# fabioiuri/DRecPy

Hardware: AMD Instinct MI355X
Metric: training samples/sec (user-item pairs) (higher is better)
Workload: dtype f32; 1 GPU; CDAE hidden_factors=128 sampled-output sparse-Adagrad on synth-10m-shaped synthetic (10000000 users x 1000000 items, 199573906 positives), corruption 0.2, neg_ratio 5; batch_per_gpu=65536, global_batch=65536, touch_list=prepared ahead on a side stream, batches=fresh device-sampled batch every step (sampler running ahead on the side stream)

## Files before the change

### drecpy_amd/_lib.py

```python
import ctypes as C
import os

_HERE = os.path.dirname(os.path.abspath(__file__))
LIB_PATH = os.path.join(_HERE, 'libdrx.so')

LOSS_BCE, LOSS_MSE = 0, 1
TARGETS_REFERENCE, TARGETS_PER_ROW = 0, 1
OPT_ADAM, OPT_ADAGRAD, OPT_ROWWISE_ADAGRAD = 0, 1, 2
DENSE_AUX_CLEAN = 0x100
KEY_NONE = 0xFFFFFFFF
SHARD_SELF_BYPASS = 1
BATCH_SHARE_USERS = 1


class DrxError(RuntimeError):
    pass


DRX_REC_SIGMOID_BIAS, DRX_REC_BIAS, DRX_REC_CLIP = 0, 1, 2

KNN_METRICS = {'cosine': 0, 'adjusted_cosine': 1, 'cosine_cf': 2, 'jaccard': 3, 'msd': 4, 'pearson': 5}
KNN_USER, KNN_ITEM = 0, 1
KNN_AGGREGATIONS = {'mean': 0, 'weighted_mean': 1}

# ... 69 lines not shown

class NcfDims(C.Structure):
    _fields_ = [(n, C.c_int32) for n in ('n_users', 'n_items', 'kg', 'km', 'ldg', 'ldm', 'n_layers')] + \
               [('f', C.c_int32 * 4), ('off_w', C.c_int32 * 4), ('off_b', C.c_int32 * 4), ('off_h', C.c_int32), ('off_b0', C.c_int32),
                ('n_small', C.c_int32)]


class CsrList(C.Structure):
    _fields_ = [('keys', C.c_void_p), ('T', C.c_int32), ('n_rows', C.c_int32), ('row_ptr', C.c_void_p), ('order', C.c_void_p)]


class DmfDims(C.Structure):
    _fields_ = [('n_layers', C.c_int32 * 2), ('f', (C.c_int32 * 4) * 2), ('ld0', C.c_int32 * 2),
                ('off_k', (C.c_int32 * 4) * 2), ('off_b', (C.c_int32 * 4) * 2), ('n_small', C.c_int32),
                ('l2_norm_vectors', C.c_int32), ('off_scale', C.c_int32)]


class DmfArgs(C.Structure):
    _fields_ = [(n, C.c_void_p) for n in ('K0u', 'K0i', 'sw', 'u_indptr', 'u_indices', 'u_values', 'i_indptr', 'i_indices',
                                          'i_values', 'uid', 'iid', 'y')] + [('target_mode', C.c_int32), ('y_mean', C.c_float)] + \
               [(n, C.c_void_p) for n in ('off_u', 'off_i')] + [('B', C.c_int32)] + \
               [(n, C.c_void_p) for n in ('dz0u', 'dz0i', 'tkeys_u', 'tsrc_u', 'tcoef_u', 'tkeys_i', 'tsrc_i', 'tcoef_i',
                                          'gsw_part', 'loss_part', 'pred_out', 'rep_u_out', 'rep_i_out', 'work', 'inv_u', 'inv_i',
                                          'gptr_u', 'gptr_i', 'grows_u', 'grows_i')] + [('n_du', C.c_int32), ('n_di', C.c_int32)] + \
               [(n, C.c_void_p) for n in ('map_u', 'map_i', 'rho_u', 'rho_i')] + [('stamp', C.c_uint32)] + \
               [(n, C.c_void_p) for n in ('nd_dev', 'y_mean_dev', 'work_order')] + [('n_work', C.c_int32), ('seg_len', C.c_int32)] + \
               [(n, C.c_void_p) for n in ('zseg', 'zpart', 'n_work_dev')]


class DmfK0Update(C.Structure):
    _fields_ = [(n, C.c_void_p) for n in ('K0u', 'm_u', 'v_u', 'K0i', 'm_i', 'v_i')] + [('n_items', C.c_int32), ('n_users', C.c_int32)] + \
               [(n, C.c_float) for n in ('alpha_u', 'alpha_i', 'l2_coef', 'beta1', 'beta2', 'eps')] + [('row_order', C.c_void_p), ('n_long', C.c_int32), ('opt_kind', C.c_int32)]


class Optim(C.Structure):
    _fields_ = [('kind', C.c_int32), ('lr', C.c_float), ('reg_rate', C.c_float), ('beta1', C.c_float),
                ('beta2', C.c_float), ('eps', C.c_float), ('alpha', C.c_float * 5),
                ('s1', C.c_void_p * 5), ('s2', C.c_void_p * 5)]


_lib = None

SIGNATURES = {
    'drx_version': (C.c_int, []),
    'drx_strerror': (C.c_char_p, [C.c_int]),
    'drx_hash_u32': (C.c_uint32, [C.c_uint64, C.c_uint32, C.c_uint32]),
    'drx_event_create': (C.c_void_p, []),
    'drx_event_destroy': (None, [C.c_void_p]),
    'drx_event_record': (C.c_int, [C.c_void_p, C.c_void_p]),
    'drx_stream_wait_event': (C.c_int, [C.c_void_p, C.c_void_p]),
    'drx_event_synchronize': (C.c_int, [C.c_void_p]),
    'drx_stream_create_cu_slice': (C.c_void_p, [C.c_int32]),
    'drx_stream_destroy': (None, [C.c_void_p]),
    'drx_cdae_forward': (C.c_int, [C.POINTER(CdaeParams), C.POINTER(History), C.POINTER(Batch), C.c_void_p,
                                   C.c_void_p, C.c_void_p]),
    'drx_cdae_scratch_bytes': (C.c_size_t, [C.POINTER(CdaeParams), C.c_int32, C.c_int32, C.c_int32]),
    'drx_cdae_step_dense': (C.c_int, [C.POINTER(CdaeParams), C.POINTER(Optim), C.POINTER(History), C.POINTER(Batch),
                                      C.c_int32, C.c_int32, C.c_void_p, C.c_size_t, C.c_void_p, C.c_void_p]),
    'drx_cdae_step_sparse': (C.c_int, [C.POINTER(CdaeParams), C.POINTER(Optim), C.POINTER(History), C.POINTER(Batch),
                                       C.c_int32, C.c_void_p, C.c_size_t, C.c_void_p, C.c_void_p]),
    'drx_cdae_step_sparse_timed': (C.c_int, [C.POINTER(CdaeParams), C.POINTER(Optim), C.POINTER(History),
                                             C.POINTER(Batch), C.c_int32, C.c_void_p, C.c_size_t, C.c_void_p,
                                             C.POINTER(C.c_void_p), C.c_void_p]),
    'drx_cdae_prep_bytes': (C.c_size_t, [C.POINTER(CdaeParams), C.c_int32, C.c_int32]),
    'drx_cdae_sparse_prepare': (C.c_int, [C.POINTER(CdaeParams), C.POINTER(History), C.POINTER(Batch), C.c_void_p,
                                          C.c_size_t, C.c_void_p]),
    'drx_cdae_step_sparse_prepared': (C.c_int, [C.POINTER(CdaeParams), C.POINTER(Optim), C.POINTER(History),
                                                C.POINTER(Batch), C.c_int32, C.c_void_p, C.c_size_t, C.c_void_p,
                                                C.c_size_t, C.c_void_p, C.POINTER(C.c_void_p), C.c_void_p]),
    'drx_cdae_prep_bytes_hot': (C.c_size_t, [C.POINTER(CdaeParams), C.c_int32, C.c_int32, C.c_int32]),
    'drx_cdae_scratch_bytes_hot': (C.c_size_t, [C.POINTER(CdaeParams), C.c_int32, C.c_int32, C.c_int32]),
    'drx_cdae_sparse_prepare_hot': (C.c_int, [C.POINTER(CdaeParams), C.POINTER(History), C.POINTER(Batch), C.POINTER(HotHead),
                                              C.c_void_p, C.c_size_t, C.c_void_p]),
    'drx_debug_prep_counts': (C.c_int, [C.POINTER(CdaeParams), C.POINTER(History), C.POINTER(Batch), C.POINTER(HotHead), C.c_void_p,
                                        C.c_int32, C.c_int32, C.c_int32, C.c_void_p, C.c_size_t, C.c_void_p, C.c_void_p, C.c_void_p,
                                        C.c_void_p, C.c_void_p, C.POINTER(C.c_int32), C.c_void_p]),
    'drx_debug_prep_result': (C.c_int, [C.POINTER(CdaeParams), C.c_int32, C.c_int32, C.c_int32, C.c_void_p, C.c_size_t, C.c_void_p,
                                        C.c_void_p, C.c_void_p, C.c_void_p, C.c_void_p, C.c_void_p]),
    'drx_debug_cdae_reduce': (C.c_int, [C.POINTER(CdaeParams), C.POINTER(Optim), C.POINTER(History), C.POINTER(Batch), C.POINTER(HotHead),
                                        C.c_void_p, C.c_size_t, C.c_void_p, C.c_void_p, C.c_void_p, C.c_int32, C.c_void_p, C.c_size_t,
                                        C.c_void_p]),
    'drx_debug_span_plan': (C.c_int, [C.POINTER(CdaeParams), C.c_int32, C.c_int32, C.c_int32, C.c_void_p, C.c_size_t, C.c_void_p,
                                      C.c_void_p, C.c_void_p, C.c_void_p]),
    'drx_cdae_step_sparse_hot': (C.c_int, [C.POINTER(CdaeParams), C.POINTER(Optim), C.POINTER(History), C.POINTER(Batch),
                                           C.POINTER(HotHead), C.c_int32, C.c_void_p, C.c_size_t, C.c_void_p, C.c_size_t,
                                           C.c_void_p, C.POINTER(C.c_void_p), C.c_void_p]),
    'drx_cdae_hot_rows_for': (C.c_int32, [C.POINTER(CdaeParams), C.c_int32, C.c_int32, C.c_int32, C.c_int32]),
    'drx_cdae_prep_forget': (None, [C.c_void_p]),
    'drx_point_sample_scratch_bytes': (C.c_size_t, [C.c_int32]),
    'drx_list_sample_device': (C.c_int, [C.POINTER(ListGroups), C.c_int32, C.c_int32, C.c_int32, C.c_int32, C.c_uint64, C.c_void_p, C.c_void_p,
                                         C.c_void_p, C.c_void_p]),
    'drx_point_sample': (C.c_int, [C.POINTER(History), C.c_int32, C.c_int32, C.c_int32, C.c_int32, C.c_uint64,
                                   C.c_void_p, C.c_void_p, C.c_void_p, C.c_void_p, C.c_void_p, C.c_size_t, C.c_void_p, C.c_uint32,
                                   C.c_void_p]),
    'drx_point_sample_recorded': (C.c_int, [C.POINTER(History), C.POINTER(History), C.c_int32, C.c_int32, C.c_int32, C.c_int32, C.c_uint64,
                                   C.c_void_p, C.c_void_p, C.c_void_p, C.c_void_p, C.c_void_p, C.c_size_t, C.c_void_p, C.c_uint32,
                                   C.c_void_p]),
    'drx_point_sample_by_user_scratch_bytes': (C.c_size_t, [C.c_int32, C.c_int32]),
    'drx_point_sample_by_user': (C.c_int, [C.POINTER(History), C.POINTER(History), C.c_int32, C.c_int32, C.c_int32, C.c_int32, C.c_uint64,
                                           C.c_void_p, C.c_void_p, C.c_void_p, C.c_void_p, C.c_void_p, C.c_size_t, C.c_void_p, C.c_uint32,
                                           C.c_void_p]),
    'drx_point_sample_valued': (C.c_int, [C.POINTER(History), C.POINTER(History), C.c_void_p, C.c_float, C.c_float, C.c_int32, C.c_int32,
                                          C.c_int32, C.c_int32, C.c_uint64, C.c_void_p, C.c_void_p, C.c_void_p, C.c_void_p]),
    'drx_dmf_distinct_scratch_bytes': (C.c_size_t, [C.c_int32, C.c_int32, C.c_int32]),
    'drx_dmf_batch_distinct_device': (C.c_int, [C.c_void_p, C.c_void_p, C.c_void_p, C.c_int32, C.c_int32, C.c_int32] + [C.c_void_p] * 10 +
                                      [C.c_void_p, C.c_size_t, C.c_void_p]),
    'drx_shard_prep_bytes': (C.c_size_t, [C.POINTER(CdaeParams), C.POINTER(Shard), C.c_int32, C.c_int32]),
    'drx_shard_work_bytes': (C.c_size_t, [C.POINTER(Shard)]),
    'drx_shard_prep_layout': (C.c_int, [C.POINTER(CdaeParams), C.POINTER(Shard), C.c_int32, C.c_int32, C.POINTER(C.c_size_t)]),
    'drx_shard_prepare': (C.c_int, [C.POINTER(CdaeParams), C.POINTER(Shard), C.POINTER(History), C.POINTER(Batch), C.c_void_p,
                                    C.c_size_t, C.c_void_p, C.c_size_t, C.c_void_p]),
    'drx_shard_owner_table_bytes': (C.c_size_t, [C.POINTER(Shard), C.c_int32]),
    'drx_shard_chunks': (C.c_int32, [C.POINTER(Shard)]),
    'drx_shard_unit_shift': (C.c_int32, [C.POINTER(Shard)]),
    'drx_shard_owner_index': (C.c_int, [C.POINTER(Shard), C.c_void_p, C.c_int32, C.POINTER(C.c_int32), C.c_int32, C.c_int32, C.c_void_p,
                                        C.c_size_t, C.c_void_p]),
    'drx_shard_gather_rows': (C.c_int, [C.POINTER(CdaeParams), C.POINTER(Shard), C.c_void_p, C.c_int32, C.POINTER(C.c_int32),
                                        C.c_int32, C.c_void_p, C.c_void_p]),
    'drx_shard_step_scratch_bytes': (C.c_size_t, [C.POINTER(CdaeParams), C.c_int32, C.c_int32]),
    'drx_shard_step_local': (C.c_int, [C.POINTER(CdaeParams), C.POINTER(Optim), C.POINTER(Shard), C.POINTER(History), C.POINTER(Batch),
                                       C.c_void_p, C.c_size_t, C.c_void_p, C.c_void_p, C.c_int32, C.c_int32, C.c_void_p, C.c_size_t,
                                       C.POINTER(C.c_void_p), C.c_void_p]),
    'drx_shard_apply': (C.c_int, [C.POINTER(CdaeParams), C.POINTER(Optim), C.POINTER(Shard), C.c_int32, C.c_void_p, C.c_void_p,
                                  C.c_int32, C.POINTER(C.c_int32), C.c_int32, C.c_int32, C.c_void_p, C.POINTER(C.c_void_p), C.POINTER(C.c_int64),
                                  C.c_void_p, C.c_void_p]),
    'drx_shard_exchange_sizes': (C.c_int, [C.POINTER(CdaeParams), C.POINTER(Shard), C.c_void_p, C.c_void_p, C.POINTER(C.c_int64)]),
    'drx_shard_phase_layout': (C.c_int, [C.POINTER(CdaeParams), C.POINTER(Shard), C.c_void_p, C.c_void_p, C.c_int32, C.POINTER(C.c_int64)]),
    'drx_shard_phase_keys': (C.c_int, [C.POINTER(Shard), C.c_void_p, C.POINTER(ShardExchange), C.c_void_p]),
    'drx_shard_phase_rows': (C.c_int, [C.POINTER(CdaeParams), C.POINTER(Shard), C.c_void_p, C.POINTER(ShardExchange), C.c_int32, C.c_void_p]),
    'drx_shard_phase_local': (C.c_int, [C.POINTER(CdaeParams), C.POINTER(Optim), C.POINTER(Shard), C.POINTER(History), C.POINTER(Batch),
                                        C.c_void_p, C.POINTER(ShardExchange), C.c_void_p, C.c_size_t, C.c_int32, C.c_int32, C.c_void_p,
                                        C.c_size_t, C.POINTER(C.c_void_p), C.c_void_p]),
    'drx_shard_phase_tail': (C.c_int, [C.POINTER(CdaeParams), C.POINTER(Optim), C.POINTER(Shard), C.c_void_p, C.POINTER(ShardExchange),
                                       C.POINTER(ShardExchange), C.c_int32, C.c_void_p, C.c_void_p]),
    'drx_copy_f4': (C.c_int, [C.c_void_p, C.c_void_p, C.c_size_t, C.c_void_p]),
    'drx_copy_f4_variant': (C.c_int, [C.c_void_p, C.c_void_p, C.c_size_t, C.c_int32, C.c_void_p]),
    'drx_comm_unique_id': (C.c_int, [C.c_void_p]),
    'drx_comm_create': (C.c_int, [C.c_void_p, C.c_int32, C.c_int32, C.c_uint32, C.POINTER(C.c_void_p)]),
    'drx_comm_destroy': (C.c_int, [C.c_void_p]),
    'drx_comm_stream': (C.c_void_p, [C.c_void_p]),
    'drx_comm_alltoallv': (C.c_int64, [C.c_void_p, C.c_void_p, C.POINTER(C.c_int64), C.POINTER(C.c_int64), C.c_void_p, C.POINTER(C.c_int64),
                                       C.POINTER(C.c_int64), C.c_void_p]),
    'drx_comm_wait': (C.c_int, [C.c_void_p, C.c_int64, C.c_void_p]),
    'drx_comm_last_error': (C.c_char_p, []),
    'drx_adam_dense': (C.c_int, [C.c_void_p, C.c_void_p, C.c_void_p, C.c_void_p, C.c_int64, C.c_float, C.c_float, C.c_float,
                                 C.c_float, C.c_float, C.c_void_p]),
    'drx_scatter_scratch_bytes': (C.c_size_t, [C.c_int32, C.c_int32, C.c_int32]),
    'drx_scatter_rows': (C.c_int, [C.c_void_p, C.c_int32, C.c_void_p, C.c_void_p, C.c_void_p, C.c_void_p, C.c_int32,
                                   C.c_int32, C.c_void_p, C.c_void_p, C.c_void_p, C.c_size_t, C.c_void_p]),
    'drx_batch_offsets': (C.c_int, [C.c_void_p, C.c_void_p, C.c_int32, C.c_void_p, C.c_void_p, C.c_size_t, C.c_void_p]),
    'drx_sumsq': (C.c_int, [C.c_void_p, C.c_int64, C.c_void_p, C.c_int32, C.c_void_p]),
    'drx_rows_dot': (C.c_int, [C.c_void_p, C.c_int32, C.c_void_p, C.c_int32, C.c_int32, C.c_void_p, C.c_void_p,
                               C.c_void_p]),
    'drx_adam_segments': (C.c_int, [C.c_void_p, C.c_void_p, C.c_void_p, C.c_void_p, C.POINTER(AdamSegments), C.c_float,
                                    C.c_float, C.c_float, C.c_void_p]),
    'drx_caser_grid': (C.c_int, [C.POINTER(CaserDims), C.c_int32]),
    'drx_caser_fwd_bwd': (C.c_int, [C.POINTER(CaserDims), C.POINTER(CaserArgs), C.c_void_p, C.c_void_p]),
    'drx_caser_step_small': (C.c_int, [C.POINTER(CaserDims), C.POINTER(CaserArgs), C.c_void_p, C.c_void_p, C.c_void_p, C.c_void_p,
                                       C.POINTER(AdamSegments), C.c_float, C.c_float, C.c_float, C.c_void_p]),
    'drx_caser_hidden': (C.c_int, [C.POINTER(CaserDims), C.POINTER(CaserArgs), C.c_void_p]),
    'drx_rows_csr_adam_multi': (C.c_int, [C.POINTER(CsrAdamTable), C.c_int32, C.c_float, C.c_float, C.c_float, C.c_void_p]),
    'drx_dmf_grid': (C.c_int, [C.c_int32]),
    'drx_dmf_work_bytes': (C.c_size_t, [C.c_int32]),
    'drx_dmf_fwd_bwd': (C.c_int, [C.POINTER(DmfDims), C.POINTER(DmfArgs), C.c_void_p, C.c_void_p]),
    'drx_dmf_step_small': (C.c_int, [C.POINTER(DmfDims), C.POINTER(DmfArgs), C.c_void_p, C.c_void_p, C.c_void_p, C.c_void_p,
                                     C.POINTER(AdamSegments), C.c_float, C.c_float, C.c_float, C.c_void_p]),
# ... 217 lines not shown
```

### drecpy_amd/csrc/drx_cdae.hip

```cpp
#include "drx_common.hpp"
#include "drx_rows.hpp"
#include "drx_segreduce.hpp"
#include <cstring>
#include "drx_scan.hpp"
#include "drx_prep.hpp"
#include "drx_segstream.hpp"
#include "drx_cdae_host.hpp"
#include <type_traits>
#include <mutex>
#include <unordered_map>

#ifdef DRX_STAMPS
static unsigned long long *h_stamps = nullptr;
extern "C" int drx_debug_set_stamps(unsigned long long *buf, unsigned int) { h_stamps = buf; return 0; }
#endif

namespace drx {

struct SparseBufs {
  float *dz1;
  float *g2;
  float *dz2;
  float *lossb;
  float *phead, *ptail;
  float *phs, *pts;
  float *pblock, *pbs;
  float *bpart;
  const uint8_t *solo_v, *solo_o;
  unsigned long long *stamps;
  const int32_t *order;
  const int32_t *usamp, *worder, *n_items;
  const WorkItem *witem;
  int T, n_chunks, n_bpart;
};

template <int G, int J, int KIND = -1>
__device__ __forceinline__ void sparse_apply(const DrxCdaeParams &P, const DrxOptim &opt, int B, uint32_t key, int lane,
                                             const float4 (&g)[J], float gs) {
  const uint32_t N = (uint32_t)P.n_items;
  float *const tW = P.W, *const tO = P.W2T, *const tV = P.V;
  float *const a0 = opt.s1[0], *const a1 = opt.s1[1], *const a2 = opt.s1[2];
  float *const c0 = opt.s2[0], *const c1 = opt.s2[1], *const c2 = opt.s2[2];
  const int var = key < N ? 0 : (key < 2 * N ? 1 : 2);
  const size_t row = key - (uint32_t)var * N;
  float *const tab = var == 0 ? tW : (var == 1 ? tO : tV);
  float *const s1 = var == 0 ? a0 : (var == 1 ? a1 : a2);
  float *const s2 = var == 0 ? c0 : (var == 1 ? c1 : c2);
  OptScalars o = opt_for(opt, 0, B);
  o.inv_k = 1.0f / (float)P.k;
  float4 w[J];
  load_row<G, J>(tab, row, P.ld, lane, w);
  row_update<G, J, KIND>(o, tab, s1, s2, row, P.ld, lane, w, g);
  if (var == 1 && lane == 0) {
    const int kind = KIND >= 0 ? KIND : o.kind;
    float pb = P.b2[row], m = opt.s1[4][row], v = kind == DRX_OPT_ADAM ? opt.s2[4][row] : 0.f;
    o.rb = 0.f;
    opt_update1<KIND>(o, gs, pb, m, v);
    P.b2[row] = pb; opt.s1[4][row] = m;
    if (kind == DRX_OPT_ADAM) opt.s2[4][row] = v;
  }
}

template <int G, int J>
__device__ __forceinline__ float sampled_hidden(const DrxCdaeParams &P, const DrxBatch &bt, float scale, int b, int lane,
                                                const float4 (&acc)[J], float4 (&h)[J], float4 (&w2)[J]) {
  hidden_act<G, J>(P, bt.uid[b], scale, lane, acc, h);
  load_row<G, J>(P.W2T, (size_t)bt.iid[b], P.ld, lane, w2);
  float d = 0.f;
#pragma unroll
  for (int j = 0; j < J; ++j) d += f4_dot(w2[j], h[j]);
  return group_sum<G>(d);
}

template <int G, int J, int KIND = -1>
__device__ __forceinline__ void sampled_rest(const DrxCdaeParams &P, const DrxOptim &opt, const DrxHistory &H, const DrxBatch &bt,
                                             float scale, uint32_t qthr, int loss_kind, const SparseBufs &S, int b, int lane,
                                             float d, const float4 (&h)[J], const float4 (&w2)[J],
                                             float4 (*dz1_out)[J] = nullptr) {
  const int u = bt.uid[b], i = bt.iid[b];
  const float y = bt.y[b];
  const float p = sigmoidf_(d + P.b2[i]);
  const float invB = 1.0f / (float)bt.B;
  float lval, dp;
  if (loss_kind == DRX_LOSS_BCE) { lval = bce_elem(y, p); dp = bce_grad(y, p) * invB; }
  else { lval = (p - y) * (p - y); dp = 2.0f * (p - y) * invB; }
  const float dz2 = dp * p * (1.0f - p);
  float4 dz1[J], g2[J];
#pragma unroll
  for (int j = 0; j < J; ++j) {
    dz1[j].x = dz2 * w2[j].x * h[j].x * (1.0f - h[j].x); dz1[j].y = dz2 * w2[j].y * h[j].y * (1.0f - h[j].y);
    dz1[j].z = dz2 * w2[j].z * h[j].z * (1.0f - h[j].z); dz1[j].w = dz2 * w2[j].w * h[j].w * (1.0f - h[j].w);
    g2[j].x = dz2 * h[j].x; g2[j].y = dz2 * h[j].y; g2[j].z = dz2 * h[j].z; g2[j].w = dz2 * h[j].w;
  }
  store_row<G, J>(S.dz1, (size_t)b, P.ld, lane, dz1);
  if (lane == 0) S.lossb[b] = lval;
  const uint8_t *const pv = S.solo_v, *const po = S.solo_o;
  const bool solo_v = pv && pv[b], solo_o = po && po[b];
  if (solo_o) {
    sparse_apply<G, J, KIND>(P, opt, bt.B, (uint32_t)P.n_items + (uint32_t)i, lane, g2, dz2);
  } else {
    store_row<G, J>(S.g2, (size_t)b, P.ld, lane, g2);
    if (lane == 0) S.dz2[b] = dz2;
  }
  if (solo_v) sparse_apply<G, J, KIND>(P, opt, bt.B, 2u * (uint32_t)P.n_items + (uint32_t)u, lane, dz1, 0.f);
  if (dz1_out) {
#pragma unroll
    for (int j = 0; j < J; ++j) (*dz1_out)[j] = dz1[j];
  }
}

template <int G, int J, int KIND = -1>
__device__ __forceinline__ void sampled_finish(const DrxCdaeParams &P, const DrxOptim &opt, const DrxHistory &H, const DrxBatch &bt,
                                               float scale, uint32_t qthr, int loss_kind, const SparseBufs &S, int b, int lane,
                                               const float4 (&acc)[J]) {
  float4 h[J], w2[J];
#ifdef DRX_STAMPS
  if (acc[0].x == acc[0].x) DRX_STAMP(S.stamps, b, 5, lane);
#endif
  const float d = sampled_hidden<G, J>(P, bt, scale, b, lane, acc, h, w2);
#ifdef DRX_STAMPS
  if (d == d) DRX_STAMP(S.stamps, b, 6, lane);
#endif
  sampled_rest<G, J, KIND>(P, opt, H, bt, scale, qthr, loss_kind, S, b, lane, d, h, w2);
  DRX_STAMP(S.stamps, b, 7, lane);
}

template <int G, int J>
__global__ __launch_bounds__(kBlock) void k_kshard_fwd(DrxCdaeParams P, DrxHistory H, DrxBatch bt, float scale, uint32_t qthr,
                                                       float *__restrict__ h_out, float *__restrict__ dot_out,
                                                       const int32_t *__restrict__ order) {
  const int lane = threadIdx.x % G;
  const int slot = blockIdx.x * (kBlock / G) + threadIdx.x / G;
  if (slot >= bt.B) return;
  const int b = order ? order[slot] : slot;
  float4 acc[J], h[J], w2[J];
  DenseAux none{};
  gather_bag<G, J, 0>(P, H, bt, qthr, b, lane, acc, none, nullptr, nullptr, 0);
  const float d = sampled_hidden<G, J>(P, bt, scale, b, lane, acc, h, w2);
  store_row<G, J>(h_out, (size_t)b, P.ld, lane, h);
  if (lane == 0) dot_out[b] = d;
}

// ... 156 lines not shown
      for (int wv = 0; wv < n_waves; ++wv) {
        float4 x[J];
        load_row<G, J>(lds, (size_t)(wv * RT + t), P.ld, lane, x);
#pragma unroll
        for (int j = 0; j < J; ++j) f4_add(acc[j], x[j]);
      }
      float4 brow[J];
      load_row<G, J>(P.b, 0, P.ld, lane, brow);
      hidden_act_rows<G, J>(P, scale, lane, acc, vrow, brow, h);
      load_row<G, J>(P.W2T, (size_t)bt.iid[b], P.ld, lane, w2);
      float d = 0.f;
#pragma unroll
      for (int j = 0; j < J; ++j) d += f4_dot(w2[j], h[j]);
      d = group_sum<G>(d);
      sampled_rest<G, J, KIND>(P, opt, H, bt, scale, qthr, loss_kind, S, b, lane, d, h, w2, &dz1);
#pragma unroll
      for (int j = 0; j < J; ++j) f4_add(dsum[j], dz1[j]);
    }
  }
  __syncthreads();
  if (r < n) store_row<G, J>(lds, (size_t)r, P.ld, lane, dsum);
  __syncthreads();
  if (r == 0) {
    float4 t[J];
#pragma unroll
    for (int j = 0; j < J; ++j) t[j] = f4_zero();
    for (int rr = 0; rr < min(n, R); ++rr) {
      float4 x[J];
      load_row<G, J>(lds, (size_t)rr, P.ld, lane, x);
#pragma unroll
      for (int j = 0; j < J; ++j) f4_add(t[j], x[j]);
    }
    store_row<G, J>(S.dz1, (size_t)bt.B + w, P.ld, lane, t);
  }
}

template <int G, int J>
__global__ __launch_bounds__(kBlock) void k_sampled_fwd_bwd_wg(DrxCdaeParams P, DrxOptim opt, DrxHistory H, DrxBatch bt, float scale,
                                                               uint32_t qthr, int loss_kind, SparseBufs S) {
  extern __shared__ __align__(16) float lds[];
  constexpr int R = kBlock / G;
  const int lane = threadIdx.x % G, r = threadIdx.x / G;
  const int b = blockIdx.x;
  float4 acc[J];
  DenseAux none{};
  gather_bag<G, J, 0>(P, H, bt, qthr, b, lane, acc, none, nullptr, nullptr, 0, r, R);
  store_row<G, J>(lds, (size_t)r, P.ld, lane, acc);
  __syncthreads();
  if (r != 0) return;
#pragma unroll
  for (int j = 0; j < J; ++j) acc[j] = f4_zero();
#pragma unroll 8
  for (int rr = 0; rr < R; ++rr) {
    float4 v[J];
    load_row<G, J>(lds, (size_t)rr, P.ld, lane, v);
#pragma unroll
    for (int j = 0; j < J; ++j) f4_add(acc[j], v[j]);
  }
  sampled_finish<G, J>(P, opt, H, bt, scale, qthr, loss_kind, S, b, lane, acc);
}

template <int KIND>
struct DirectPolicyT {
  DrxCdaeParams P;
  DrxOptim opt;
  int B;
  float scale;
  const float *dz1;
  long long g2_off;
  const float *dz2;
  template <int G, int J>
  __device__ __forceinline__ void load(uint32_t key, uint32_t bv, int lane, float4 (&row)[J], float &sc, float &coef) const {
    const uint32_t N = (uint32_t)P.n_items;
    const bool is_out = key >= N && key < 2 * N;
    const uint32_t b = bv & 0x7FFFFFFFu;
    load_row<G, J>(dz1 + (is_out ? g2_off : 0ll), (size_t)b, P.ld, lane, row);
    if (is_out) sc = dz2[b];
    coef = key < N ? ((bv >> 31) ? -scale : scale) : 1.0f;
  }
  template <int G, int J>
  __device__ __forceinline__ void finish(uint32_t key, int, int lane, const float4 (&g)[J], float gs) const {
    sparse_apply<G, J, KIND>(P, opt, B, key, lane, g, gs);
  }
  static constexpr bool kStreamParks = false;
  __device__ __forceinline__ StreamArrays stream_arrays() const {
    const uint32_t N = (uint32_t)P.n_items;
    return StreamArrays{{0u, N, 2u * N}, {dz1, dz1 + g2_off, dz1}, {P.W, P.W2T, P.V}, {opt.s1[0], opt.s1[1], opt.s1[2]},
                        {scale, 1.0f, 1.0f}, {nullptr, dz2, nullptr}, {nullptr, P.b2, nullptr}, {nullptr, opt.s1[4], nullptr}};
  }
  __device__ __forceinline__ float stream_decay() const { return opt.reg_rate / (float)B; }
  __device__ __forceinline__ void stream_update(float g, float &p, float &a) const {
    static_assert(KIND == DRX_OPT_ADAGRAD || KIND < 0, "one slot per element");
    OptScalars o = opt_for(opt, 0, B);
    float unused = 0.f;
    opt_update1<DRX_OPT_ADAGRAD>(o, g, p, a, unused);
  }
  __device__ __forceinline__ void stream_update_scalar(float g, float &p, float &a) const { stream_update(g, p, a); }
};
using DirectPolicy = DirectPolicyT<-1>;
using DirectPolicyAdagrad = DirectPolicyT<DRX_OPT_ADAGRAD>;

template <int G, int J, int NT>
__device__ __forceinline__ void bias_final_body(const DrxCdaeParams &P, const DrxOptim &opt, const BiasArgs &A,
                                                float *lds , float *red) {
  constexpr int R = NT / G;
  const int lane = threadIdx.x % G, r = threadIdx.x / G;
  float4 acc[J];
#pragma unroll
  for (int j = 0; j < J; ++j) acc[j] = f4_zero();
  constexpr int NB = J == 1 ? 8 : 2;
  for (int i = r; i < A.n_part; i += NB * R) {
    float4 v[NB][J];
#pragma unroll
    for (int q = 0; q < NB; ++q) {
#pragma unroll
      for (int j = 0; j < J; ++j) v[q][j] = f4_zero();
      if (i + q * R < A.n_part) load_row<G, J>(A.part, (size_t)(i + q * R), P.ld, lane, v[q]);
    }
#pragma unroll
    for (int q = 0; q < NB; ++q)
#pragma unroll
      for (int j = 0; j < J; ++j) f4_add(acc[j], v[q][j]);
  }
  store_row<G, J>(lds, (size_t)r, P.ld, lane, acc);
  __syncthreads();
  if (r == 0) {
    float4 g[J], w[J];
#pragma unroll
    for (int j = 0; j < J; ++j) g[j] = f4_zero();
#pragma unroll 8
    for (int rr = 0; rr < R; ++rr) {
      float4 v[J];
      load_row<G, J>(lds, (size_t)rr, P.ld, lane, v);
#pragma unroll
      for (int j = 0; j < J; ++j) f4_add(g[j], v[j]);
    }
    load_row<G, J>(P.b, 0, P.ld, lane, w);
    OptScalars o = opt_for(opt, 0, A.B);
    if (o.kind == DRX_OPT_ROWWISE_ADAGRAD) o.kind = DRX_OPT_ADAGRAD;
    o.rb = 0.f;
    row_update<G, J>(o, P.b, opt.s1[3], opt.s2[3], 0, P.ld, lane, w, g);
  }
  if (A.loss_out) {
    const float *lp = A.part + (size_t)A.n_part * P.ld;
    float a = 0.f;
    for (int b = threadIdx.x; b < A.n_part; b += NT) a += lp[b];
    float t = block_sum(a, red);
    if (threadIdx.x == 0) { A.loss_out[0] = t / (float)A.B; A.loss_out[1] = 0.f; }
  }
}

template <int G, int J>
struct BiasFinalExtra {
  DrxCdaeParams P;
  DrxOptim opt;
  BiasArgs A;
  __device__ __forceinline__ void operator()(float *lds) const {
    __shared__ float red[kFixBlock / 64];
    bias_final_body<G, J, kFixBlock>(P, opt, A, lds, red);
  }
};

constexpr int kHotSlice = 512;
constexpr int kHotGroup = 64;

struct HotArgs {
  const float *dz1;
  const uint32_t *mask;
  float *part;
  uint32_t *any;
  const int32_t *item;
  float scale;
  int B, H, Bw, S, first;
  float *bpart;
  const float *lossb;
};

static inline int hot_slices(int B) { return (B + kHotSlice - 1) / kHotSlice; }
static inline int hot_groups(int H) { return (H + kHotGroup - 1) / kHotGroup; }

typedef __bf16 hot_bf16x8 __attribute__((ext_vector_type(8)));
typedef float hot_f32x4 __attribute__((ext_vector_type(4)));
typedef uint32_t hot_u32x4 __attribute__((ext_vector_type(4)));

template <int LD, int NT>
struct HotPartialExtra {
  HotArgs A;
  __device__ __forceinline__ void operator()(float *) const {
    constexpr int CS = LD / 16, NW = NT / 64;
    const int lane = threadIdx.x & 63, wv = __builtin_amdgcn_readfirstlane((int)(threadIdx.x >> 6));
    const int ngr = (A.H + kHotGroup - 1) / kHotGroup;
    const int task = ((int)blockIdx.x - A.first) * NW + wv;
    if (task >= A.S * ngr * CS) return;
    const int cs = task % CS, rg = (task / CS) % ngr, s = task / (CS * ngr);
    const int c = lane & 15, kq = lane >> 4;
    const int nt = min(kHotGroup, A.H - rg * kHotGroup) / 16;
    const int b_begin = s * kHotSlice, b_end = min(A.B, b_begin + kHotSlice);
    const uint32_t *const mgrp = A.mask + (size_t)rg * kHotGroup * A.Bw;
    const float *const slice = A.dz1 + (size_t)b_begin * LD + cs * 16;
    const uint32_t mlane = (uint32_t)c * (uint32_t)A.Bw, xlane = (uint32_t)(8 * kq * LD + c);
    hot_f32x4 acc[4];
#pragma unroll
    for (int t = 0; t < 4; ++t) acc[t] = hot_f32x4{0.f, 0.f, 0.f, 0.f};
    uint32_t seen = 0u;
    float bsum = 0.f;
    for (int b0 = b_begin; b0 < b_end; b0 += 32) {
      float x[8];
      uint32_t w[4];
      {
        const float *const rows = slice + (size_t)(b0 - b_begin) * LD;
        const uint32_t *const words = mgrp + (b0 >> 5);
        const int left = A.B - b0 - 8 * kq;
        if (left >= 8) {
#pragma unroll
          for (int j = 0; j < 8; ++j) x[j] = rows[xlane + (uint32_t)(j * LD)];
        } else {
#pragma unroll
          for (int j = 0; j < 8; ++j) x[j] = j < left ? rows[xlane + (uint32_t)(j * LD)] : 0.f;
        }
#pragma unroll
        for (int t = 0; t < 4; ++t) w[t] = (words + (size_t)(16 * min(t, nt - 1)) * A.Bw)[mlane] & (t < nt ? ~0u : 0u);
      }
      hot_u32x4 bh, bm, bl;
#pragma unroll
      for (int i = 0; i < 4; ++i) {
        uint32_t hv[2], mv[2], lv[2];
#pragma unroll
        for (int e = 0; e < 2; ++e) {
          const float v = x[2 * i + e];
          bsum += v;
          hv[e] = __float_as_uint(v) & 0xFFFF0000u;
          const float r1 = v - __uint_as_float(hv[e]);
          mv[e] = __float_as_uint(r1) & 0xFFFF0000u;
          lv[e] = __float_as_uint(r1 - __uint_as_float(mv[e])) & 0xFFFF0000u;
        }
        bh[i] = (hv[0] >> 16) | hv[1];
        bm[i] = (mv[0] >> 16) | mv[1];
        bl[i] = (lv[0] >> 16) | lv[1];
      }
#pragma unroll
      for (int t = 0; t < 4; ++t) {
        seen |= (w[t] != 0u ? 1u : 0u) << t;
        const uint32_t bits = (w[t] >> (8 * kq)) & 0xFFu;
        hot_u32x4 a;
#pragma unroll
        for (int i = 0; i < 4; ++i) a[i] = ((bits >> (2 * i)) & 1u) * 0x3F80u | ((bits >> (2 * i + 1)) & 1u) * 0x3F800000u;
        const hot_bf16x8 av = __builtin_bit_cast(hot_bf16x8, a);
        acc[t] = __builtin_amdgcn_mfma_f32_16x16x32_bf16(av, __builtin_bit_cast(hot_bf16x8, bh), acc[t], 0, 0, 0);
        acc[t] = __builtin_amdgcn_mfma_f32_16x16x32_bf16(av, __builtin_bit_cast(hot_bf16x8, bm), acc[t], 0, 0, 0);
        acc[t] = __builtin_amdgcn_mfma_f32_16x16x32_bf16(av, __builtin_bit_cast(hot_bf16x8, bl), acc[t], 0, 0, 0);
      }
    }
    float *const out = A.part + ((size_t)s * A.H + rg * kHotGroup) * LD + cs * 16 + c;
#pragma unroll
    for (int t = 0; t < 4; ++t)
      if (t < nt) {
#pragma unroll
        for (int i = 0; i < 4; ++i) out[(size_t)(16 * t + 4 * kq + i) * LD] = acc[t][i];
      }
    if (cs == 0) {
      uint32_t rows[4];
#pragma unroll
      for (int t = 0; t < 4; ++t) rows[t] = (uint32_t)__ballot((seen >> t) & 1u) & 0xFFFFu;
      if (lane == 0) {
        uint32_t *const any = A.any + (size_t)s * (A.H / 32) + rg * (kHotGroup / 32);
        any[0] = rows[0] | (rows[1] << 16);
        if (nt > 2) any[1] = rows[2] | (rows[3] << 16);
      }
    }
    if (rg == 0) {
      const float g1 = __shfl(bsum, c + 16, 64), g2 = __shfl(bsum, c + 32, 64), g3 = __shfl(bsum, c + 48, 64);
      if (kq == 0) A.bpart[(size_t)s * LD + cs * 16 + c] = ((bsum + g1) + g2) + g3;
      if (cs == 0 && A.lossb) {
        float l = 0.f;
        for (int b = b_begin + lane; b < b_end; b += 64) l += A.lossb[b];
#pragma unroll
        for (int o = 32; o > 0; o >>= 1) l += __shfl_xor(l, o, 64);
        if (lane == 0) A.bpart[(size_t)A.S * LD + s] = l;
      }
    }
  }
};

template <int LD, class Policy>
struct HotFinishExtra {
  HotArgs A;
  Policy pol;
  __device__ __forceinline__ void operator()(float *lds) const {
    constexpr int NT = kFixBlock, NQ = NT / LD;
    static_assert(NQ >= 1 && NT % LD == 0, "a row per workgroup");
    const int h = (int)blockIdx.x - A.first;
    if (h >= A.H) return;
    const uint32_t bit = 1u << (h & 31);
    bool touched = false;
    for (int s = (int)threadIdx.x; s < A.S; s += NT) touched |= (A.any[(size_t)s * (A.H / 32) + (h >> 5)] & bit) != 0u;
    if (!__syncthreads_or(touched)) return;
    const int c = (int)threadIdx.x % LD, q = (int)threadIdx.x / LD;
    const int per = (A.S + NQ - 1) / NQ, s0 = q * per, s1 = min(A.S, s0 + per);
    float sum = 0.f;
#pragma unroll 8
    for (int s = s0; s < s1; ++s) sum += A.part[((size_t)s * A.H + h) * LD + c];
    lds[q * LD + c] = sum;
    __syncthreads();
    if (q == 0) {
      float t = lds[c];
#pragma unroll
      for (int k = 1; k < NQ; ++k) t += lds[k * LD + c];
      const StreamArrays SA = pol.stream_arrays();
      const size_t off = (size_t)A.item[h] * LD + c;
      float pv = SA.table[0][off], av = SA.slot[0][off];
      pol.stream_update(fmaf(pol.stream_decay(), pv, A.scale * t), pv, av);
      SA.table[0][off] = pv;
      SA.slot[0][off] = av;
    }
  }
};

template <class E1, class E2>
struct ExtraPair {
  E1 e1;
  int n1;
  E2 e2;
  __device__ __forceinline__ void operator()(float *lds) const {
    if ((int)blockIdx.x < n1) e1(lds);
    else e2(lds);
  }
};

static SparseBufs sparse_layout(Carver &cv, const DrxCdaeParams &P, int B, int n_touch_slots) {
  SparseBufs S{};
  S.T = n_touch_slots + 2 * B;
  const int chunk = seg_chunk(long_segments(S.T, P));
  S.n_chunks = (S.T + chunk - 1) / chunk;
  S.n_bpart = 1024;
  S.dz1 = cv.take<float>((size_t)2 * B * P.ld);
  S.g2 = cv.take<float>((size_t)B * P.ld);
  S.dz2 = cv.take<float>(B);
  S.lossb = cv.take<float>(B);
  S.phead = cv.take<float>((size_t)S.n_chunks * P.ld);
  S.ptail = cv.take<float>((size_t)S.n_chunks * P.ld);
  S.phs = cv.take<float>(S.n_chunks);
  S.pts = cv.take<float>(S.n_chunks);
  {
    const int cpb = kSegBlock / pick_geom(P.ld).G;
    const int n_blocks = (S.n_chunks + cpb - 1) / cpb;
    S.pblock = cv.take<float>((size_t)n_blocks * P.ld);
    S.pbs = cv.take<float>(n_blocks);
  }
  S.bpart = cv.take<float>((size_t)S.n_bpart * (P.ld + 1));
  return S;
}

static std::mutex g_hot_mu;
static std::unordered_map<const void *, int> g_hot_of;
static void hot_record(const void *prepared, int H) {
  std::lock_guard<std::mutex> lk(g_hot_mu);
  if (H > 0) g_hot_of[prepared] = H;
  else g_hot_of.erase(prepared);
}
static int hot_recorded(const void *prepared) {
  std::lock_guard<std::mutex> lk(g_hot_mu);
  const auto it = g_hot_of.find(prepared);
  return it == g_hot_of.end() ? 0 : it->second;
}

struct HotBufs { float *part; uint32_t *any; float *bpart; };
static HotBufs hot_layout(Carver &cv, const DrxCdaeParams &P, int B, int H) {
  HotBufs HB{nullptr, nullptr, nullptr};
  if (H <= 0) return HB;
  HB.part = cv.take<float>((size_t)hot_slices(B) * H * P.ld);
  HB.any = cv.take<uint32_t>((size_t)hot_slices(B) * (H / 32));
  HB.bpart = cv.take<float>((size_t)hot_slices(B) * (P.ld + 1));
  return HB;
}

template <int G, int J>
static void launch_forward(ForwardForm form, const DrxCdaeParams &P, const DrxOptim &opt, const DrxHistory &hist, const DrxBatch &bt,
                           float scale, uint32_t qthr, int32_t loss_kind, const SparseBufs &S, const float *ks_h, const float *ks_dot,
                           hipStream_t st) {
  constexpr int gpb = kBlock / G;
  const dim3 groups((bt.B + gpb - 1) / gpb);
  const bool adagrad = opt.kind == DRX_OPT_ADAGRAD;
  switch (form) {
  case ForwardForm::ColumnShard:
    hipLaunchKernelGGL((k_kshard_rest<G, J>), groups, dim3(kBlock), 0, st, P, opt, hist, bt, scale, qthr, loss_kind, S, ks_h, ks_dot);
    break;
  case ForwardForm::SharedUsers:
    if constexpr (G >= 16 && J <= 2) {
      const long long wmax = (long long)(P.n_users < bt.B ? P.n_users : bt.B) + bt.B / share_item_triples(P.ld) + 1;
      hipLaunchKernelGGL((adagrad ? k_items_fwd_bwd<G, J, DRX_OPT_ADAGRAD> : k_items_fwd_bwd<G, J>), dim3((unsigned)(wmax < bt.B ? wmax : bt.B)),
                         dim3(kItemThreads), share_item_lds_bytes(P.ld), st, P, opt, hist, bt, scale, qthr, loss_kind, S);
    }
    break;
  case ForwardForm::PerWorkgroup:
    hipLaunchKernelGGL((k_sampled_fwd_bwd_wg<G, J>), dim3(bt.B), dim3(kBlock), (size_t)gpb * P.ld * 4, st, P, opt, hist, bt, scale, qthr,
                       loss_kind, S);
    break;
  case ForwardForm::PerGroup:
    hipLaunchKernelGGL((adagrad ? k_sampled_fwd_bwd<G, J, DRX_OPT_ADAGRAD> : k_sampled_fwd_bwd<G, J>), groups, dim3(kBlock), 0, st, P, opt, hist,
                       bt, scale, qthr, loss_kind, S);
    break;
  }
}

template <int G, int J, class Policy>
static int reduce_and_finish(ReduceForm form, const DrxCdaeParams &P, const DrxOptim &opt, const SparseBufs &S, const SegBufs &SB,
                             const PlanBufs &PB, const SpanPlan &plan, const BiasArgs &BA, const HotArgs &HA, void *const *events,
                             hipStream_t st) {
  const Policy pol{P, opt, BA.B, HA.scale, S.dz1, (long long)(S.g2 - S.dz1), S.dz2};
  const BiasFinalExtra<G, J> bias{P, opt, BA};
  int rc = DRX_EINVAL;
  if (HA.H == 0) rc = launch_reduce<G, J>(form, SB, PB, plan, pol, BA, st);
  else if constexpr (kHotBuilt<G, J, Policy>) {
    constexpr int NT = kStreamThreads<G>;
    HotArgs part = HA;
    part.first = 0;
    const int n_hot = (HA.S * hot_groups(HA.H) * (G / 4) + NT / 64 - 1) / (NT / 64);
    rc = launch_reduce_streamed<G, J>(SB, PB, plan, pol, n_hot, HotPartialExtra<4 * G, NT>{part}, st);
  }
  if (rc) return rc;
  DRX_HIP(phase_event(events, 3, st));
  rc = DRX_EINVAL;
  if (HA.H == 0) rc = launch_spans<G, J>(SB, PB, plan, pol, 1, bias, st);
  else if constexpr (kHotBuilt<G, J, Policy>) {
    HotArgs fin = HA;
    fin.first = kSpanBlocks + 1;
    using Finish = ExtraPair<BiasFinalExtra<G, J>, HotFinishExtra<4 * G, Policy>>;
    rc = launch_spans<G, J>(SB, PB, plan, pol, 1 + HA.H, Finish{bias, fin.first, {fin, pol}}, st);
  }
  if (rc) return rc;
  DRX_HIP(phase_event(events, 4, st));
  DRX_HIP(phase_event(events, 5, st));
  return DRX_OK;
}

}

using namespace drx;

extern "C" {

size_t drx_cdae_scratch_bytes(const DrxCdaeParams *p, int32_t B, int32_t n_touch_slots, int32_t dense_mode) {
  if (!p || B < 1 || n_touch_slots < 0) return 0;
  Carver c(nullptr, 0);
  if (dense_mode) {
    c.off = dense_layout_bytes(*p, B);
  } else {
    (void)sparse_layout(c, *p, B, n_touch_slots);
    (void)prep_layout(c, *p, B, n_touch_slots);
  }
  return align_up(c.off, 256) + 256;
}

struct GivenGradients { const float *dz1, *g2, *dz2; int32_t form; };

static int step_sparse_impl(const DrxCdaeParams *p, const DrxOptim *opt, const DrxHistory *hist, const DrxBatch *bt,
                            int32_t loss_kind, const void *prepared, size_t prepared_bytes, void *scratch, size_t scratch_bytes,
                            float *loss_out, void *const *events, void *stream, const float *ks_h = nullptr,
                            const float *ks_dot = nullptr, const DrxHotHead *hot = nullptr, const GivenGradients *given = nullptr) {
  int rc = check_params(p);
  if (rc) return rc;
  rc = check_batch(hist, bt);
  if (rc || !opt || !scratch || !bt->iid || (!bt->y && !given) || !bt->keep_off) return DRX_EINVAL;
  if (opt->kind != DRX_OPT_ADAM && opt->kind != DRX_OPT_ADAGRAD && opt->kind != DRX_OPT_ROWWISE_ADAGRAD) return DRX_EINVAL;
  for (int i = 0; i < 5; ++i)
    if (!opt->s1[i] || (opt->kind == DRX_OPT_ADAM && !opt->s2[i])) return DRX_EINVAL;
  if ((uint64_t)2 * p->n_items + p->n_users + 1 >= 0xFFFFFFFFull) return DRX_EINVAL;
  hipStream_t st = (hipStream_t)stream;
  const int H = hot ? hot->H : 0;
  if (prepared && hot_recorded(prepared) != H) return DRX_EINVAL;
  Carver cv(scratch, scratch_bytes);
  SparseBufs S = sparse_layout(cv, *p, bt->B, bt->n_touch_slots);
  const HotBufs HB = hot_layout(cv, *p, bt->B, H);
  PrepBufs R{};
  if (prepared) {
    Carver cp(const_cast<void *>(prepared), prepared_bytes);
    R = prep_layout(cp, *p, bt->B, bt->n_touch_slots, H);
    if (!cp.ok()) return DRX_ESCRATCH;
  } else {
    R = prep_layout(cv, *p, bt->B, bt->n_touch_slots, H);
  }
  if (!cv.ok()) return DRX_ESCRATCH;
  const float scale = 1.0f / (1.0f - bt->q);
  const uint32_t qthr = q_threshold(bt->q);
  const int rows_per_block = (bt->B + S.n_bpart - 1) / S.n_bpart;
  const int n_bpart = (bt->B + rows_per_block - 1) / rows_per_block;
  S.solo_v = prepared ? R.solo_v : nullptr;
  S.solo_o = prepared ? R.solo_o : nullptr;
  S.order = prepared ? R.order : nullptr;
  SegBufs SB{R.keys_s, R.vals_s, S.phead, S.ptail, S.phs, S.pts, nullptr, nullptr, nullptr, nullptr, S.T, S.n_chunks, p->ld, nullptr};
#ifdef DRX_STAMPS
  S.stamps = SB.stamps = h_stamps;
#endif
  PlanBufs PB{S.pblock, S.pbs};
  if (prepared && ks_h && share_users(p, hist, bt, R)) return DRX_EINVAL;
  const bool share = prepared && !ks_h && share_users(p, hist, bt, R);
  S.usamp = share ? R.usamp : nullptr;
  S.witem = share ? R.witem : nullptr;
  S.worder = share ? R.worder : nullptr;
  S.n_items = share ? R.n_du : nullptr;
  ReduceForm form = reduce_form(opt->kind, bt->B, S.T, *p);
  const ForwardForm fwd = forward_form(ks_h != nullptr, share, bt->B, bt->n_touch_slots);
  if (H > 0 && !hot_head_fits(form, p->ld, share, ks_h != nullptr)) return DRX_EINVAL;
  if (given) {
    if (share || (given->form == 1 && (H > 0 || form == ReduceForm::PlannedLong))) return DRX_EINVAL;
    if (given->form == 1) form = ReduceForm::PlannedShort;
  }
  const HotArgs HA{S.dz1, R.hmask, HB.part, HB.any, hot ? hot->item : nullptr, scale, bt->B, H, R.Bw, hot_slices(bt->B), 0, HB.bpart,
                   loss_out ? S.lossb : nullptr};
// ... 169 lines not shown

int drx_debug_prep_counts(const DrxCdaeParams *p, const DrxHistory *hist, const DrxBatch *bt, const DrxHotHead *hot, uint8_t *present,
                          int32_t ipr, int32_t cshift, int32_t world, void *prepared, size_t prepared_bytes, uint32_t *hist_out,
                          uint32_t *buckets_out, uint32_t *keys_out, uint32_t *vals_out, uint32_t *mask_out, int32_t *info_out,
                          void *stream) {
  int rc = check_params(p);
  if (rc) return rc;
  rc = check_batch(hist, bt);
  if (rc || !prepared || !bt->iid || !bt->keep_off || !hist_out || !buckets_out || !keys_out || !vals_out || !info_out) return DRX_EINVAL;
  if ((uint64_t)2 * p->n_items + p->n_users + 1 >= 0xFFFFFFFFull) return DRX_EINVAL;
  if (hot && !hot_ok(p, hot)) return DRX_EINVAL;
  if (present && (ipr < 1 || cshift < 0 || cshift > 30 || world < 1)) return DRX_EINVAL;
  const int H = hot ? hot->H : 0;
  if (H > 0 && !mask_out) return DRX_EINVAL;
  Carver cp(prepared, prepared_bytes);
  const PrepBufs R = prep_layout(cp, *p, bt->B, bt->n_touch_slots, H);
  if (!cp.ok()) return DRX_ESCRATCH;
  if (H > 0 && !hot_list_fits(R.T, *p, present != nullptr)) return DRX_EINVAL;
  hipStream_t st = (hipStream_t)stream;
  hot_record(prepared, 0);
  launch_touches(p, hist, bt, R, st, TouchPresence{present, WireGeo{present ? ipr : 1, present ? cshift : 0, present ? world : 1}},
                 H > 0 ? hot->slot : nullptr, H > 0 ? hot->item : nullptr);
  const SortRider rider{bt->keep_off, bt->B, R.order_work, R.partials, R.partial_rows};
  const uint32_t *h = nullptr;
  rc = sort_first_counts(R.sort_temp, R.sort_bytes, R.keys, (size_t)R.T, R.bits, true, st, rider, &h);
  if (rc) return rc;
  const int dbits = sort_first_digit_bits(R.bits);
  DRX_HIP(hipMemcpyAsync(hist_out, h, sizeof(uint32_t) << dbits, hipMemcpyDeviceToDevice, st));
  DRX_HIP(hipMemcpyAsync(buckets_out, R.order_work, 256 * sizeof(uint32_t), hipMemcpyDeviceToDevice, st));
  DRX_HIP(hipMemcpyAsync(keys_out, R.keys, (size_t)R.T * sizeof(uint32_t), hipMemcpyDeviceToDevice, st));
  DRX_HIP(hipMemcpyAsync(vals_out, R.vals, (size_t)R.T * sizeof(uint32_t), hipMemcpyDeviceToDevice, st));
  if (H > 0) DRX_HIP(hipMemcpyAsync(mask_out, R.hmask, (size_t)H * R.Bw * sizeof(uint32_t), hipMemcpyDeviceToDevice, st));
  info_out[0] = dbits;
  info_out[1] = R.partials ? R.partial_rows : 0;
  info_out[2] = R.T;
  info_out[3] = DRX_PREP_ROUNDS ? touch_grid(bt->B) : (bt->B + 15) / 16;
  DRX_LAUNCH_CHECK();
  return DRX_OK;
}

int drx_debug_prep_result(const DrxCdaeParams *p, int32_t B, int32_t n_touch_slots, int32_t H, const void *prepared, size_t prepared_bytes,
                          uint32_t *keys_s_out, uint32_t *vals_s_out, uint8_t *solo_v_out, uint8_t *solo_o_out, int32_t *order_out,
                          void *stream) {
  int rc = check_params(p);
  if (rc) return rc;
  if (B < 1 || n_touch_slots < 0 || hot_rows(p, H) < 0 || !prepared || !keys_s_out || !vals_s_out || !solo_v_out || !solo_o_out || !order_out)
    return DRX_EINVAL;
  Carver cp(const_cast<void *>(prepared), prepared_bytes);
  const PrepBufs R = prep_layout(cp, *p, B, n_touch_slots, H);
  if (!cp.ok()) return DRX_ESCRATCH;
  hipStream_t st = (hipStream_t)stream;
  DRX_HIP(hipMemcpyAsync(keys_s_out, R.keys_s, (size_t)R.T * sizeof(uint32_t), hipMemcpyDeviceToDevice, st));
  DRX_HIP(hipMemcpyAsync(vals_s_out, R.vals_s, (size_t)R.T * sizeof(uint32_t), hipMemcpyDeviceToDevice, st));
  DRX_HIP(hipMemcpyAsync(solo_v_out, R.solo_v, (size_t)B, hipMemcpyDeviceToDevice, st));
  DRX_HIP(hipMemcpyAsync(solo_o_out, R.solo_o, (size_t)B, hipMemcpyDeviceToDevice, st));
  DRX_HIP(hipMemcpyAsync(order_out, R.order, (size_t)B * sizeof(int32_t), hipMemcpyDeviceToDevice, st));
  return DRX_OK;
}

int drx_debug_cdae_reduce(const DrxCdaeParams *p, const DrxOptim *opt, const DrxHistory *hist, const DrxBatch *bt, const DrxHotHead *hot,
                          const void *prepared, size_t prepared_bytes, const float *dz1_in, const float *g2_in, const float *dz2_in,
                          int32_t form, void *scratch, size_t scratch_bytes, void *stream) {
  if (!dz1_in || !g2_in || !dz2_in || (form != 0 && form != 1) || (hot && !hot_ok(p, hot))) return DRX_EINVAL;
  const GivenGradients given{dz1_in, g2_in, dz2_in, form};
  return step_sparse_impl(p, opt, hist, bt, DRX_LOSS_BCE, prepared, prepared_bytes, scratch, scratch_bytes, nullptr, nullptr, stream,
                          nullptr, nullptr, hot && hot->H > 0 ? hot : nullptr, &given);
}

int drx_debug_span_plan(const DrxCdaeParams *p, int32_t B, int32_t n_touch_slots, int32_t H, const void *prepared, size_t prepared_bytes,
                        uint8_t *ext_out, uint32_t *desc_out, uint32_t *cnt_out, void *stream) {
  int rc = check_params(p);
  if (rc) return rc;
  if (B < 1 || n_touch_slots < 0 || hot_rows(p, H) < 0 || !prepared || !ext_out || !desc_out || !cnt_out) return DRX_EINVAL;
  Carver cp(const_cast<void *>(prepared), prepared_bytes);
  const PrepBufs R = prep_layout(cp, *p, B, n_touch_slots, H);
  if (!cp.ok()) return DRX_ESCRATCH;
  hipStream_t st = (hipStream_t)stream;
  DRX_HIP(hipMemcpyAsync(ext_out, R.plan.ext, (size_t)R.n_chunks, hipMemcpyDeviceToDevice, st));
  DRX_HIP(hipMemcpyAsync(desc_out, R.plan.desc, (size_t)R.n_chunks * sizeof(uint2), hipMemcpyDeviceToDevice, st));
  DRX_HIP(hipMemcpyAsync(cnt_out, R.plan.cnt, 2 * sizeof(uint32_t), hipMemcpyDeviceToDevice, st));
  return DRX_OK;
}

int drx_cdae_step_sparse_hot(const DrxCdaeParams *p, const DrxOptim *opt, const DrxHistory *hist, const DrxBatch *bt,
                             const DrxHotHead *hot, int32_t loss_kind, const void *prepared, size_t prepared_bytes, void *scratch,
                             size_t scratch_bytes, float *loss_out, void *const *events, void *stream) {
  if (!hot_ok(p, hot)) return DRX_EINVAL;
  return step_sparse_impl(p, opt, hist, bt, loss_kind, prepared, prepared_bytes, scratch, scratch_bytes, loss_out, events, stream,
                          nullptr, nullptr, hot);
}

int32_t drx_cdae_hot_rows_for(const DrxCdaeParams *p, int32_t opt_kind, int32_t B, int32_t n_touch_slots, int32_t H) {
  if (B < 1 || n_touch_slots < 0 || hot_rows(p, H) <= 0) return 0;
  return hot_head_fits(reduce_form(opt_kind, B, n_touch_slots + 2 * B, *p), p->ld, false, false) ? H : 0;
}

void drx_cdae_prep_forget(const void *prepared) {
  if (prepared) hot_record(prepared, 0);
}

}
```

### drecpy_amd/csrc/drx_common.hpp

```cpp
#pragma once
#include <cstring>
#include <hip/hip_runtime.h>
#include <stdint.h>
#include "drx.h"

#define DRX_HIP(expr)                                  \
  do {                                                 \
    hipError_t e_ = (expr);                            \
    if (e_ != hipSuccess) return (int)e_;              \
  } while (0)

#define DRX_LAUNCH_CHECK()                             \
  do {                                                 \
    hipError_t e_ = hipGetLastError();                 \
    if (e_ != hipSuccess) return (int)e_;              \
  } while (0)

namespace drx {

constexpr int kWave = 64;
constexpr int kBlock = 256;

__host__ __device__ inline uint32_t hash_u32(uint64_t seed, uint32_t a, uint32_t b) {
  uint64_t x = seed + (uint64_t)a * 0x9E3779B97F4A7C15ull + (uint64_t)b * 0xD1B54A32D192ED03ull;
// ... 1 lines not shown
  x ^= x >> 27; x *= 0x94D049BB133111EBull;
  x ^= x >> 31;
  return (uint32_t)(x >> 32);
}

__host__ __device__ inline uint32_t q_threshold(float q) {
  double t = (double)q * 4294967296.0;
  if (t <= 0.0) return 0u;
  if (t >= 4294967295.0) return 0xFFFFFFFFu;
  return (uint32_t)t;
}

template <int G>
__device__ __forceinline__ float group_sum(float v) {
#pragma unroll
  for (int m = G / 2; m >= 1; m >>= 1) v += __shfl_xor(v, m, kWave);
  return v;
}

__device__ __forceinline__ float4 f4_zero() { return make_float4(0.f, 0.f, 0.f, 0.f); }
__device__ __forceinline__ void f4_fma(float4 &a, float s, const float4 &x) {
  a.x = fmaf(s, x.x, a.x); a.y = fmaf(s, x.y, a.y); a.z = fmaf(s, x.z, a.z); a.w = fmaf(s, x.w, a.w);
}
__device__ __forceinline__ void f4_add(float4 &a, const float4 &x) {
  a.x += x.x; a.y += x.y; a.z += x.z; a.w += x.w;
}
__device__ __forceinline__ float f4_dot(const float4 &a, const float4 &b) {
  return fmaf(a.x, b.x, fmaf(a.y, b.y, fmaf(a.z, b.z, a.w * b.w)));
}

__device__ __forceinline__ float sigmoidf_(float x) { return 1.0f / (1.0f + expf(-x)); }

__device__ __forceinline__ float bce_elem(float t, float p) {
  const float eps = 1e-7f;
  float pc = fminf(fmaxf(p, eps), 1.0f - eps);
  return -(t * logf(pc + eps) + (1.0f - t) * logf(1.0f - pc + eps));
}
__device__ __forceinline__ float bce_grad(float t, float p) {
  const float eps = 1e-7f;
  float pc = fminf(fmaxf(p, eps), 1.0f - eps);
  float g = -(t / (pc + eps) - (1.0f - t) / (1.0f - pc + eps));
  return (p >= eps && p <= 1.0f - eps) ? g : 0.0f;
}

struct Geom { int G, J; };
inline Geom pick_geom(int ld) {
  if (ld <= 16) return {4, 1};
  if (ld <= 32) return {8, 1};
  if (ld <= 64) return {16, 1};
  if (ld <= 128) return {32, 1};
  if (ld <= 256) return {64, 1};
  if (ld <= 512) return {64, 2};
  return {64, 4};
}

template <int G_, int J_> struct GeomT { static constexpr int G = G_, J = J_; };

template <class F>
inline int dispatch_geom(int ld, F &&f) {
  const Geom g = pick_geom(ld);
  if (g.G == 4) return f(GeomT<4, 1>{});
  if (g.G == 8) return f(GeomT<8, 1>{});
  if (g.G == 16) return f(GeomT<16, 1>{});
  if (g.G == 32) return f(GeomT<32, 1>{});
  if (g.J == 1) return f(GeomT<64, 1>{});
  if (g.J == 2) return f(GeomT<64, 2>{});
  return f(GeomT<64, 4>{});
}

__device__ __forceinline__ void wave_lds_sync() {
  __builtin_amdgcn_fence(__ATOMIC_RELEASE, "workgroup");
  __builtin_amdgcn_wave_barrier();
  __builtin_amdgcn_fence(__ATOMIC_ACQUIRE, "workgroup");
}

#ifdef DRX_STAMPS
#define DRX_STAMP(buf, unit, i, lane)                                                             \
  do {                                                                                            \
    if ((lane) == 0 && (buf) && (unsigned)(unit) < 110000u) (buf)[(size_t)(unit) * 16 + (i)] = wall_clock64(); \
  } while (0)
#else
#define DRX_STAMP(buf, unit, i, lane) do { } while (0)
#endif

inline size_t align_up(size_t x, size_t a) { return (x + a - 1) / a * a; }

struct Carver {
  char *base; size_t off; size_t cap;
  Carver(void *p, size_t c) : base((char *)p), off(0), cap(c) {}
  template <typename T> T *take(size_t n) {
    off = align_up(off, 256);
    T *r = (T *)(base ? base + off : nullptr);
    off += n * sizeof(T);
    return r;
  }
  bool ok() const { return off <= cap; }
};

size_t sort_pairs_temp_bytes(size_t n, int end_bit);
int sort_pairs(void *temp, size_t temp_bytes, const uint32_t *kin, uint32_t *kout, const uint32_t *vin,
               uint32_t *vout, size_t n, int end_bit, hipStream_t stream);
__device__ __forceinline__ int degree_bucket(const int32_t *keep_off, int b) {
  const int d = (keep_off[b + 1] - keep_off[b]) >> 2;
  return 255 - (d > 255 ? 255 : d);
}

__device__ __forceinline__ unsigned long long same_bucket_lanes(bool valid, int d) {
  unsigned long long m = __ballot(valid);
#pragma unroll
  for (int bit = 0; bit < 8; ++bit) {
    const bool one = (d >> bit) & 1;
    const unsigned long long bl = __ballot(one);
    m &= one ? bl : ~bl;
  }
  return m;
}

template <int NT>
__device__ __forceinline__ void degree_counts_body(const int32_t *__restrict__ keep_off, int B, unsigned int *__restrict__ work, int block_id,
                                                   unsigned int *cnt ) {
  for (int i = threadIdx.x; i < 256; i += NT) cnt[i] = 0;
  __syncthreads();
  const int b = block_id * NT + (int)threadIdx.x, lane = threadIdx.x & 63;
  const bool valid = b < B;
  const int d = valid ? degree_bucket(keep_off, b) : 0;
  const unsigned long long m = same_bucket_lanes(valid, d);
  if (valid && lane == __ffsll((long long)m) - 1) atomicAdd(&cnt[d], (unsigned int)__popcll(m));
  __syncthreads();
  for (int i = threadIdx.x; i < 256; i += NT)
    if (cnt[i]) atomicAdd(&work[i], cnt[i]);
}

struct SortRider {
  const int32_t *keep_off;
  int B;
  unsigned int *counts;
  const uint32_t *partials = nullptr;
  int partial_rows = 0;
};
constexpr int kPartialWords = 512;
int sort_first_digit_bits(int end_bit);

int sort_pairs_ex(void *temp, size_t temp_bytes, const uint32_t *kin, uint32_t *kout, const uint32_t *vin, uint32_t *vout, size_t n, int end_bit,
                  bool drop_none, hipStream_t stream, bool pre_zeroed = false, SortRider rider = SortRider{nullptr, 0, nullptr});
void sort_pairs_zero_region(void *temp, size_t n, int end_bit, uint32_t **words, size_t *n_words);
int sort_first_counts(void *temp, size_t temp_bytes, const uint32_t *kin, size_t n, int end_bit, bool drop_none, hipStream_t stream,
                      SortRider rider, const uint32_t **hist);

inline int bits_for(uint64_t max_key_exclusive) {
  int b = 1;
  while (b < 32 && (1ull << b) < max_key_exclusive) ++b;
  return b;
}

}
```

### drecpy_amd/csrc/drx_prep.hpp

```cpp
#pragma once
#include <algorithm>
#include "drx_common.hpp"
#include "drx_rows.hpp"
#include "drx_segreduce.hpp"
#include "drx_scan.hpp"

namespace drx {

struct WireGeo {
  int ipr, cshift, world;
  __host__ __device__ __forceinline__ uint32_t wire(int item, int is_out) const {
    const int o = item / ipr;
    const uint32_t l = 2u * (uint32_t)(item - o * ipr) + (uint32_t)(is_out ? 1 : 0);
    return (((l >> cshift) * (uint32_t)world + (uint32_t)o) << cshift) | (l & ((1u << cshift) - 1u));
  }
  __host__ __device__ __forceinline__ uint32_t local(uint32_t w) const {
    return (((w >> cshift) / (uint32_t)world) << cshift) | (w & ((1u << cshift) - 1u));
  }
  __host__ __device__ __forceinline__ uint32_t unit(uint32_t w) const { return w >> cshift; }
};

struct TouchPresence {
  uint8_t *present;
  WireGeo G;
// ... 388 lines not shown
constexpr int kLongBlocks = 256, kShortBlocks = 1024;

struct __attribute__((aligned(32))) WorkItem { int32_t p0, n, user, deg; long long hist_start, pad_; };

struct PrepBufs {
  uint32_t *keys_s, *vals_s, *keys, *vals;
  void *sort_temp;
  size_t sort_bytes;
  uint8_t *solo_v, *solo_o;
  SpanPlan plan;
  int32_t *order;
  int32_t *usamp;
  int32_t *pitem;
  WorkItem *witem;
  int32_t *worder;
  int32_t *n_du;
  unsigned int *order_work;
  int n_chunks;
  size_t result_bytes;
  int T, bits;
  uint32_t *hmask;
  int H, Bw;
  uint32_t *partials;
  int partial_rows;
};

static inline bool long_segments(int T, const DrxCdaeParams &P) { return (int64_t)T > 8 * ((int64_t)2 * P.n_items + P.n_users); }

#ifndef DRX_STREAM_DEPTH
#define DRX_STREAM_DEPTH 4
#endif
constexpr int kStreamDepth = DRX_STREAM_DEPTH;
constexpr int kStreamIndexBits = 28;
constexpr int kHotMaxG = 32;

enum class ReduceForm { Streamed, PlannedLong, PlannedShort };

template <class Policy> struct PolicyKind;
template <template <int> class PolicyT, int KIND> struct PolicyKind<PolicyT<KIND>> { static constexpr int value = KIND; };
template <int G, int J, class Policy>
constexpr bool kStreamBuilt = kStreamDepth > 0 && J == 1 && G >= 16 && PolicyKind<Policy>::value == DRX_OPT_ADAGRAD;
template <int G, int J, class Policy>
constexpr bool kHotBuilt = kStreamBuilt<G, J, Policy> && G <= kHotMaxG;

static inline ReduceForm reduce_form(int opt_kind, int B, int T, const DrxCdaeParams &K) {
  if (long_segments(T, K)) return ReduceForm::PlannedLong;
  const Geom gm = pick_geom(K.ld);
  const bool streamed = kStreamDepth > 0 && gm.J == 1 && gm.G >= 16 && K.ld == 4 * gm.G && opt_kind == DRX_OPT_ADAGRAD &&
                        B < (1 << kStreamIndexBits) && K.n_items < (1 << kStreamIndexBits) && K.n_users < (1 << kStreamIndexBits);
  return streamed ? ReduceForm::Streamed : ReduceForm::PlannedShort;
}

static inline bool hot_list_fits(int T, const DrxCdaeParams &K, bool presence) { return !presence && !long_segments(T, K); }
static inline bool hot_head_fits(ReduceForm form, int ld, bool share, bool kshard) {
  return form == ReduceForm::Streamed && pick_geom(ld).G <= kHotMaxG && !share && !kshard;
}

static inline bool forward_per_workgroup(int B, int n_touch_slots) {
  const long long mean_hist = n_touch_slots / (long long)B;
  return mean_hist > 64 || (B <= 8192 && mean_hist > 16);
}
enum class ForwardForm { ColumnShard, SharedUsers, PerWorkgroup, PerGroup };
static inline ForwardForm forward_form(bool kshard, bool share, int B, int n_touch_slots) {
  if (kshard) return ForwardForm::ColumnShard;
  if (share) return ForwardForm::SharedUsers;
  return forward_per_workgroup(B, n_touch_slots) ? ForwardForm::PerWorkgroup : ForwardForm::PerGroup;
}

static inline hipError_t phase_event(void *const *events, int i, hipStream_t st) {
  return events ? hipEventRecord((hipEvent_t)events[i], st) : hipSuccess;
}

static PrepBufs prep_layout(Carver &cv, const DrxCdaeParams &P, int B, int n_touch_slots, int H = 0) {
  PrepBufs R{};
  R.T = n_touch_slots + 2 * B;
  R.bits = bits_for((uint64_t)2 * P.n_items + P.n_users + 1);
  R.keys_s = cv.take<uint32_t>(R.T);
  R.vals_s = cv.take<uint32_t>(R.T);
  R.solo_v = cv.take<uint8_t>((size_t)2 * B);
  R.solo_o = R.solo_v ? R.solo_v + B : nullptr;
  R.plan.chunk = seg_chunk(long_segments(R.T, P));
  R.n_chunks = (R.T + R.plan.chunk - 1) / R.plan.chunk;
  R.plan.desc = cv.take<uint2>(R.n_chunks);
  R.plan.cnt = cv.take<uint32_t>(128);
  R.plan.ext = cv.take<uint8_t>(R.n_chunks);
  {
    R.plan.xstride = (R.n_chunks + 1) / 2;
    const bool placed = long_segments(R.T, P);
    const bool placed_any = placed || DRX_STREAM_PLACED != 0;
    R.plan.xrank = placed_any ? cv.take<uint32_t>((size_t)R.plan.xstride) : nullptr;
    R.plan.xperm = placed_any ? cv.take<uint32_t>((size_t)R.plan.xstride) : nullptr;
    R.usamp = placed ? cv.take<int32_t>(B) : nullptr;
    R.pitem = placed ? cv.take<int32_t>(B) : nullptr;
    R.witem = placed ? cv.take<WorkItem>((size_t)B) : nullptr;
    R.worder = placed ? cv.take<int32_t>(B) : nullptr;
    R.n_du = placed ? cv.take<int32_t>(128) : nullptr;
  }
  R.order = cv.take<int32_t>(B);
  R.result_bytes = align_up(cv.off, 256);
  R.keys = cv.take<uint32_t>(R.T);
  R.vals = cv.take<uint32_t>(R.T);
  R.sort_bytes = sort_pairs_temp_bytes(R.T, R.bits);
  R.sort_temp = cv.take<char>(R.sort_bytes);
  R.order_work = cv.take<unsigned int>(512);
  R.H = H;
  R.Bw = (B + 31) / 32;
  R.hmask = H > 0 ? cv.take<uint32_t>((size_t)H * R.Bw) : nullptr;
  R.partial_rows = DRX_PREP_ROUNDS && sort_first_digit_bits(R.bits) == 8 ? touch_grid(B) : 0;
  R.partials = R.partial_rows > 0 ? cv.take<uint32_t>((size_t)R.partial_rows * kPartialWords) : nullptr;
  return R;
}

static int plan_zero_words(const PrepBufs &R) { return (int)(((const char *)R.plan.ext + R.n_chunks - (const char *)R.plan.cnt + 3) / 4); }

static int plan_spans(const DrxCdaeParams *p, const DrxBatch *bt, const PrepBufs &R0, hipStream_t st, bool cleared) {
  const PrepBufs &R = R0;
  if (!cleared) DRX_HIP(hipMemsetAsync(R.plan.cnt, 0, (size_t)plan_zero_words(R) * 4, st));
  hipLaunchKernelGGL(k_plan_spans<0>, dim3((R.n_chunks + 255) / 256), dim3(256), 0, st, R.keys_s, R.vals_s, R.T, R.n_chunks,
                     kSegBlock / pick_geom(p->ld).G, bt->B, R.plan);
  if (R.plan.xrank) hipLaunchKernelGGL(k_place_blocks, dim3(256), dim3(256), 0, st, R.plan, R.n_chunks);
  return DRX_OK;
}

static void order_by_degree(const DrxBatch *bt, const PrepBufs &R, hipStream_t st, bool cleared) {
  if (!cleared) (void)hipMemsetAsync(R.order_work, 0, 512 * sizeof(unsigned int), st);
  const int blocks = (bt->B + 1023) / 1024;
  hipLaunchKernelGGL(k_degree_counts, dim3(blocks), dim3(1024), 0, st, bt->keep_off, bt->B, R.order_work);
  hipLaunchKernelGGL(k_degree_scatter, dim3(blocks), dim3(1024), 0, st, bt->keep_off, bt->B, R.order_work, R.order);
}

constexpr int kTpFallback = 0x7fff0001;

static __global__ __launch_bounds__(256) void k_tp_begin(DrxBatch bt, int n_users, uint32_t *__restrict__ k2, uint32_t *__restrict__ v2,
                                                         int32_t *__restrict__ se, int n_se, uint8_t *solo, uint32_t *zero_a, int n_zero_a,
                                                         uint32_t *zero_b, int n_zero_b) {
  const int tid = blockIdx.x * blockDim.x + threadIdx.x, nt = gridDim.x * blockDim.x;
  for (int j = tid; j < 2 * bt.B; j += nt) {
    k2[j] = j < bt.B ? (uint32_t)bt.uid[j] : (uint32_t)n_users + (uint32_t)bt.iid[j - bt.B];
    v2[j] = (uint32_t)j;
  }
  for (int j = tid; j < n_se; j += nt) se[j] = 0;
  for (int j = tid; j < 2 * bt.B; j += nt) solo[j] = 0;
  for (int j = tid; j < n_zero_a; j += nt) zero_a[j] = 0u;
  for (int j = tid; j < n_zero_b; j += nt) zero_b[j] = 0u;
}

static __global__ __launch_bounds__(256) void k_tp_runs(const uint32_t *__restrict__ ks, int n, int32_t *__restrict__ start, int32_t *__restrict__ end) {
  for (int p = blockIdx.x * blockDim.x + threadIdx.x; p < n; p += gridDim.x * blockDim.x) {
    const uint32_t k = ks[p];
    if (p == 0 || ks[p - 1] != k) start[k] = p;
    if (p == n - 1 || ks[p + 1] != k) end[k] = p + 1;
  }
}

#ifndef DRX_ITEM_THREADS
#define DRX_ITEM_THREADS 256
#endif
constexpr int kShareTriples = 16;
static inline int share_item_triples(int) { return kShareTriples; }
constexpr int kItemThreads = DRX_ITEM_THREADS;
static inline size_t share_item_lds_bytes(int ld) { return ((size_t)(kItemThreads / 64) * kShareTriples * ld + kShareTriples) * 4; }
static inline bool share_geometry_ok(int ld) {
  const Geom g = pick_geom(ld);
  return g.G >= 16 && g.J <= 2 && share_item_lds_bytes(ld) <= 64 * 1024;
}

// ... 301 lines not shown
```

### drecpy_amd/csrc/drx_rows.hpp

```cpp
#pragma once
#include "drx_common.hpp"

#ifndef DRX_GATHER_ROWS
#define DRX_GATHER_ROWS 8
#endif
#ifndef DRX_GATHER_PACKED
#define DRX_GATHER_PACKED 1
#endif

namespace drx {

template <int G, int J>
__device__ __forceinline__ void load_row(const float *base, size_t row, int ld, int lane, float4 (&v)[J]) {
  const float4 *r = reinterpret_cast<const float4 *>(base + row * (size_t)ld);
#pragma unroll
  for (int j = 0; j < J; ++j) {
    int c = lane + j * G;
    v[j] = (4 * c < ld) ? r[c] : f4_zero();
  }
}

template <int G, int J>
__device__ __forceinline__ void store_row(float *base, size_t row, int ld, int lane, const float4 (&v)[J]) {
  float4 *r = reinterpret_cast<float4 *>(base + row * (size_t)ld);
// ... 80 lines not shown
          tvals[touch_base + jj] = (uint32_t)b;
        }
      }
    }
    constexpr int NF = J == 1 ? DRX_GATHER_ROWS : 4;
#ifdef DRX_STAMPS
    if (first_rows && idx[0] >= -1) DRX_STAMP(stamps, b, 3, lane);
#endif
    if constexpr (DRX_GATHER_PACKED != 0 && CH <= 32) {
      uint32_t left = 0;
#pragma unroll
      for (int rr = 0; rr < IPL; ++rr) left |= (uint32_t)group_ballot<G>(kf[rr] != 0) << (rr * G);
      while (left) {
        float4 r[NF][J];
#pragma unroll
        for (int q = 0; q < NF; ++q) {
          const bool on = left != 0;
          const int tt = on ? __builtin_ctz(left) : 0;
          left &= left - 1;
          int si = idx[0];
#pragma unroll
          for (int rr = 1; rr < IPL; ++rr) si = (tt / G == rr) ? idx[rr] : si;
          const int iq = __shfl(si, tt % G, G);
#pragma unroll
          for (int jx = 0; jx < J; ++jx) r[q][jx] = f4_zero();
          if (on) load_row<G, J>(P.W, (size_t)iq, P.ld, lane, r[q]);
        }
#pragma unroll
        for (int q = 0; q < NF; ++q)
#pragma unroll
          for (int jx = 0; jx < J; ++jx) f4_add(acc[jx], r[q][jx]);
#ifdef DRX_STAMPS
        if (first_rows && acc[0].x == acc[0].x) { DRX_STAMP(stamps, b, 4, lane); first_rows = false; }
#endif
      }
    } else {
      const int n_here = (int)((e - c) < (int64_t)CH ? (e - c) : (int64_t)CH);
      for (int t = 0; t < n_here; t += NF) {
        float4 r[NF][J];
#pragma unroll
        for (int q = 0; q < NF; ++q) {
          const int tt = t + q;
          int si = idx[0], sk = kf[0];
#pragma unroll
          for (int rr = 1; rr < IPL; ++rr) { si = (tt / G == rr) ? idx[rr] : si; sk = (tt / G == rr) ? kf[rr] : sk; }
          const int iq = __shfl(si, tt % G, G);
          const int kq = (tt < n_here) ? __shfl(sk, tt % G, G) : 0;
#pragma unroll
          for (int jx = 0; jx < J; ++jx) r[q][jx] = f4_zero();
          if (kq) load_row<G, J>(P.W, (size_t)iq, P.ld, lane, r[q]);
        }
#pragma unroll
        for (int q = 0; q < NF; ++q)
#pragma unroll
          for (int jx = 0; jx < J; ++jx) f4_add(acc[jx], r[q][jx]);
#ifdef DRX_STAMPS
        if (first_rows && acc[0].x == acc[0].x) { DRX_STAMP(stamps, b, 4, lane); first_rows = false; }
#endif
      }
    }
  }
}

struct OptScalars {
  int kind;
  float lr, rb;
  float b1, b2, eps, alpha;
  float inv_k = 0.f;
};

template <int KIND = -1>
__device__ __forceinline__ void opt_update1(const OptScalars &o, float g, float &p, float &s1, float &s2) {
  const int kind = KIND >= 0 ? KIND : o.kind;
  if (kind == DRX_OPT_ADAM) {
    s1 = s1 + (g - s1) * (1.0f - o.b1);
    s2 = s2 + (g * g - s2) * (1.0f - o.b2);
    p = p - (s1 * o.alpha) / (sqrtf(s2) + o.eps);
  } else {
    s1 = s1 + g * g;
    p = p - o.lr * g / (sqrtf(s1) + o.eps);
  }
}

template <int G, int J, int KIND = -1>
__device__ __forceinline__ float row_update(const OptScalars &o, float *tab, float *s1, float *s2, size_t row, int ld,
                                            int lane, const float4 (&w)[J], const float4 (&g)[J]) {
  float sq = 0.f;
  float4 *pr = reinterpret_cast<float4 *>(tab + row * (size_t)ld);
  const int kind = KIND >= 0 ? KIND : o.kind;
  if (kind == DRX_OPT_ROWWISE_ADAGRAD) {
    float4 gg[J];
    float q = 0.f;
#pragma unroll
    for (int j = 0; j < J; ++j) {
      const float4 p = w[j];
      gg[j].x = fmaf(o.rb, p.x, g[j].x); gg[j].y = fmaf(o.rb, p.y, g[j].y);
      gg[j].z = fmaf(o.rb, p.z, g[j].z); gg[j].w = fmaf(o.rb, p.w, g[j].w);
      q += f4_dot(gg[j], gg[j]);
      sq += f4_dot(p, p);
    }
    q = group_sum<G>(q) * o.inv_k;
    const float acc = s1[row * (size_t)ld] + q;
    const float step = o.lr / (sqrtf(acc) + o.eps);
#pragma unroll
    for (int j = 0; j < J; ++j) {
      const int c = lane + j * G;
      if (4 * c < ld) {
        float4 p = w[j];
        p.x -= step * gg[j].x; p.y -= step * gg[j].y; p.z -= step * gg[j].z; p.w -= step * gg[j].w;
        pr[c] = p;
      }
    }
    if (lane == 0) s1[row * (size_t)ld] = acc;
    return sq;
  }
  float4 *a1 = reinterpret_cast<float4 *>(s1 + row * (size_t)ld);
  float4 *a2 = (kind == DRX_OPT_ADAM) ? reinterpret_cast<float4 *>(s2 + row * (size_t)ld) : nullptr;
#pragma unroll
  for (int j = 0; j < J; ++j) {
    const int c = lane + j * G;
    if (4 * c < ld) {
      float4 p = w[j];
      float4 m = a1[c];
      float4 v = a2 ? a2[c] : f4_zero();
      sq += f4_dot(p, p);
      opt_update1<KIND>(o, fmaf(o.rb, p.x, g[j].x), p.x, m.x, v.x);
      opt_update1<KIND>(o, fmaf(o.rb, p.y, g[j].y), p.y, m.y, v.y);
      opt_update1<KIND>(o, fmaf(o.rb, p.z, g[j].z), p.z, m.z, v.z);
      opt_update1<KIND>(o, fmaf(o.rb, p.w, g[j].w), p.w, m.w, v.w);
      pr[c] = p;
      a1[c] = m;
      if (a2) a2[c] = v;
    }
  }
  return sq;
}

__device__ __forceinline__ OptScalars opt_for(const DrxOptim &opt, int var, int B) {
  OptScalars o;
  o.kind = opt.kind; o.lr = opt.lr; o.rb = opt.reg_rate / (float)B;
  o.b1 = opt.beta1; o.b2 = opt.beta2; o.eps = opt.eps; o.alpha = opt.alpha[var];
  return o;
}

__device__ __forceinline__ float block_sum(float v, float *red ) {
  v = group_sum<64>(v);
  __syncthreads();
  if ((threadIdx.x & 63) == 0) red[threadIdx.x >> 6] = v;
  __syncthreads();
  float t = 0.f;
  if (threadIdx.x == 0)
    for (int i = 0; i < (int)(blockDim.x >> 6); ++i) t += red[i];
  return t;
}

}
```

### drecpy_amd/csrc/drx_segreduce.hpp

```cpp
#pragma once
#include "drx_rows.hpp"

namespace drx {

#ifndef DRX_CHUNK
#define DRX_CHUNK 32
#endif
constexpr int kChunk = DRX_CHUNK;
constexpr int kChunkLong = 64;
static inline int seg_chunk(bool long_segments) { return long_segments ? kChunkLong : kChunk; }
#ifdef DRX_SEG_WAVE_PER_CHUNK
#define SEG_GPB(G) (drx::kBlock / 64)
#else
#define SEG_GPB(G) (drx::kBlock / (G))
#endif
constexpr int kShortSpan = 64;
#ifndef DRX_SEG_BLOCK
#define DRX_SEG_BLOCK 128
#endif
constexpr int kSegBlock = DRX_SEG_BLOCK;
constexpr int kPlanShort = 16;
constexpr int kFixBlock = 512;

struct SegBufs {
// ... 37 lines not shown
#pragma unroll
    for (int r = 1; r < KPL; ++r) sel = (t / G == r) ? reg[r] : sel;
    return (uint32_t)__shfl((int)sel, t % G, G);
  };
  float4 acc[J];
#pragma unroll
  for (int jx = 0; jx < J; ++jx) acc[jx] = f4_zero();
  float accs = 0.f;
  uint32_t cur = DRX_KEY_NONE;
  int cur_pos = 0;
  bool cur_from_start = false;
  auto flush = [&](bool at_end) {
    if (cur == DRX_KEY_NONE) return;
    const bool cont_left = cur_from_start && prev_key == cur;
    const bool cont_right = at_end && next_key == cur;
    if (!cont_left && !cont_right) {
      pol.template finish<G, J>(cur, cur_pos, lane, acc, accs);
    } else if (cont_left) {
      store_row<G, J>(S.phead, (size_t)g, S.ld, lane, acc);
      if (lane == 0) S.phs[g] = accs;
    } else {
      store_row<G, J>(S.ptail, (size_t)g, S.ld, lane, acc);
      if (lane == 0) {
        S.pts[g] = accs;
        const uint32_t slot = atomicAdd(S.n_span, 1u);
        S.span_list[slot] = (uint32_t)g;
      }
    }
  };
  for (int t0 = 0; t0 < n; t0 += LB) {
    uint32_t k8[LB];
    float s8[LB], c8[LB];
    float4 rows[LB][J];
#pragma unroll
    for (int u = 0; u < LB; ++u) {
      const int t = t0 + u;
      k8[u] = t < n ? bcast(kreg, t) : DRX_KEY_NONE;
      const uint32_t b = bcast(vreg, t < n ? t : 0);
      s8[u] = 0.f;
      c8[u] = 1.f;
#pragma unroll
      for (int jx = 0; jx < J; ++jx) rows[u][jx] = f4_zero();
      if (k8[u] != DRX_KEY_NONE) pol.template load<G, J>(k8[u], b, lane, rows[u], s8[u], c8[u]);
    }
#pragma unroll
    for (int u = 0; u < LB; ++u) {
      const uint32_t key = k8[u];
      if (key != DRX_KEY_NONE) {
        if (key != cur) {
          flush(false);
          cur = key;
          cur_from_start = (t0 + u == 0);
#pragma unroll
          for (int jx = 0; jx < J; ++jx) acc[jx] = f4_zero();
          accs = 0.f;
        }
#pragma unroll
        for (int jx = 0; jx < J; ++jx) f4_fma(acc[jx], c8[u], rows[u][jx]);
        accs += s8[u];
        cur_pos = start + t0 + u;
      }
    }
  }
  const bool ran_to_end = n > 0 && bcast(kreg, n - 1) != DRX_KEY_NONE;
  flush(ran_to_end);
  if (lane == 0) {
    const uint32_t first = n > 0 ? S.keys_s[start] : DRX_KEY_NONE, last = n > 0 ? S.keys_s[end - 1] : DRX_KEY_NONE;
    const bool cont = first != DRX_KEY_NONE && first == prev_key;
    const bool middle = cont && last == first && next_key == first;
    S.cflag[g] = middle ? 2 : (cont ? 1 : 0);
  }
}

struct SpanPlan {
  uint2 *desc;
  uint32_t *cnt;
  uint8_t *ext;
  uint32_t *xrank;
  uint32_t *xperm;
  int xstride;
  int chunk;
  const int32_t *row_end;
  uint32_t row_end_keys;
};
#ifndef DRX_STREAM_PLACED
#define DRX_STREAM_PLACED 0
#endif
#ifndef DRX_XBINS
#define DRX_XBINS 8
#endif
constexpr int kXBase = 32, kXBins = DRX_XBINS;

__device__ __forceinline__ void place_block(const uint32_t *__restrict__ keys_s, const uint32_t *__restrict__ vals_s, int T, int cpb, int B,
                                            const SpanPlan &P, int blk, bool on) {
  int x = blk & (kXBins - 1);
  if (on && P.cnt[20] != 0u && (long long)blk * cpb * P.chunk >= (long long)P.cnt[20]) on = false;
  bool banded = true;
  if (on && P.chunk == kChunk) {
    const long long first = (long long)blk * cpb * P.chunk, last = first + (long long)cpb * P.chunk - 1;
    banded = first > 0 && last < T && keys_s[first] != DRX_KEY_NONE && keys_s[first - 1] == keys_s[first] && keys_s[last] == keys_s[first];
  }
  if (on && banded) {
    const int at = blk * cpb * P.chunk;
    if (at < T && keys_s[at] != DRX_KEY_NONE) {
      uint32_t b = vals_s[at];
      if (b & 0x80000000u) b &= 0x7FFFFFFFu;
      else if (b >= (uint32_t)B) b = (uint32_t)(((unsigned long long)(b - (uint32_t)B) * (unsigned long long)B) / (unsigned long long)max(1u, P.cnt[21]));
      x = (int)min((uint32_t)(kXBins - 1), (uint32_t)(((unsigned long long)b * (unsigned long long)kXBins) / (unsigned long long)(B > 0 ? B : 1)));
    }
  }
  const int lane = threadIdx.x & 63;
  unsigned long long mine = 0ull, of_lane = 0ull;
#pragma unroll
  for (int r = 0; r < kXBins; ++r) {
    const unsigned long long m = __ballot(on && x == r);
    if (x == r) mine = m;
    if (lane == r) of_lane = m;
  }
  uint32_t base = 0;
  if (lane < kXBins && of_lane) base = atomicAdd(&P.cnt[kXBase + lane], (uint32_t)__popcll(of_lane));
  base = (uint32_t)__shfl((int)base, x);
  if (on) P.xrank[blk] = ((uint32_t)x << 24) | (base + (uint32_t)__popcll(mine & ((1ull << lane) - 1ull)));
  if (on && blk == 0) { P.cnt[16] = 1u; P.cnt[17] = (uint32_t)cpb; }
}

static __global__ __launch_bounds__(256) void k_place_blocks(SpanPlan P, int n_chunks) {
  __shared__ uint32_t pre[kXBins];
  if (threadIdx.x < kXBins) {
    uint32_t run = 0;
    for (int t = 0; t < (int)threadIdx.x; ++t) run += P.cnt[kXBase + t];
    pre[threadIdx.x] = run;
  }
  __syncthreads();
  const int cpb = (int)P.cnt[17];
  const int nb = cpb > 0 ? (n_chunks + cpb - 1) / cpb : 0;
  for (int blk = blockIdx.x * blockDim.x + threadIdx.x; blk < nb; blk += gridDim.x * blockDim.x) {
    if (P.cnt[20] != 0u && (long long)blk * cpb * P.chunk >= (long long)P.cnt[20]) continue;
    const uint32_t e = P.xrank[blk];
    P.xperm[pre[e >> 24] + (e & 0xFFFFFFu)] = (uint32_t)blk;
  }
}

__device__ __forceinline__ int placed_block(const SpanPlan &P, int j, int extra, int n_wg, int cpb) {
  if (!P.xperm || P.cnt[16] == 0u || P.cnt[17] != (uint32_t)cpb) return j - extra;
  const int x = j & 7;
  int own[8], q[8], have[8], start[8];
  int run = 0;
#pragma unroll
  for (int r = 0; r < 8; ++r) {
    int c = 0;
#pragma unroll
    for (int t = 0; t < kXBins / 8; ++t) c += (int)P.cnt[kXBase + r * (kXBins / 8) + t];
    have[r] = c; start[r] = run; run += c;
    const int first = extra + ((r - extra) & 7);
    q[r] = first < extra + n_wg ? (extra + n_wg - 1 - first) / 8 + 1 : 0;
    own[r] = min(c, q[r]);
  }
  const int i = (j - (extra + ((x - extra) & 7))) / 8;
  if (i < own[x]) return (int)P.xperm[start[x] + i];
  int f = i - own[x];
#pragma unroll
  for (int r = 0; r < 8; ++r) f += r < x ? q[r] - own[r] : 0;
#pragma unroll
  for (int r = 0; r < 8; ++r) {
    const int over = have[r] - own[r];
    if (f < over) return (int)P.xperm[start[r] + own[r] + f];
    f -= over;
  }
  return -1;
}

struct PlanBufs {
  float *pblock;
  float *pbs;
};

struct SpanShape {
  int first, n_lead, n_blk, n_trail;
  __host__ __device__ SpanShape(uint2 d, int cpb) {
    const int m_in = (int)(d.y & 0x7FFFFFFFu), has_end = (int)(d.y >> 31);
    first = (int)d.x + 1;
    const int to_boundary = (cpb - first % cpb) % cpb;
    n_lead = m_in < to_boundary ? m_in : to_boundary;
    n_blk = (m_in - n_lead) / cpb;
    n_trail = m_in - n_lead - n_blk * cpb + has_end;
  }
  __host__ __device__ int total() const { return n_lead + n_blk + n_trail; }
};

__device__ __forceinline__ void plan_chunk(const uint32_t *__restrict__ keys_s, int T, int n_chunks, int cpb, const SpanPlan &P, int g) {
  const int CH = P.chunk;
  if (P.xrank && P.cnt[20] != 0u) T = min(T, (int)P.cnt[20]);
  const int start = g * CH, end = min(T, start + CH);
  if (start >= T) return;
  const uint32_t first = keys_s[start], last = keys_s[end - 1];
  const uint32_t prev = start > 0 ? keys_s[start - 1] : DRX_KEY_NONE, next = end < T ? keys_s[end] : DRX_KEY_NONE;
  const bool head_cont = first != DRX_KEY_NONE && prev == first;
  const bool tail_cont = last != DRX_KEY_NONE && next == last;
  if (!tail_cont || (head_cont && first == last)) return;
  int lo = end, hi = T;
  if (P.row_end && last < P.row_end_keys) lo = hi = P.row_end[last];
  while (lo < hi) {
    const int mid = (lo + hi) >> 1;
    if (keys_s[mid] == last) lo = mid + 1; else hi = mid;
  }
  const int seg_end = lo;
  const int full_end = seg_end / CH;
  const uint32_t m_in = (uint32_t)(full_end - (g + 1)), has_end = (seg_end % CH) ? 1u : 0u;
  if (m_in == 0) {
    P.ext[g] = (uint8_t)(seg_end - end);
    return;
  }
  const uint2 d = make_uint2((uint32_t)g, m_in | (has_end << 31));
  if (SpanShape(d, cpb).total() <= kPlanShort) P.desc[atomicAdd(&P.cnt[0], 1u)] = d;
  else P.desc[n_chunks - 1 - (int)atomicAdd(&P.cnt[1], 1u)] = d;
}

template <int DUMMY = 0>
__global__ void k_plan_spans(const uint32_t *__restrict__ keys_s, const uint32_t *__restrict__ vals_s, int T, int n_chunks, int cpb, int B,
                             SpanPlan P) {
  const int g = blockIdx.x * blockDim.x + threadIdx.x;
  if (g < n_chunks) plan_chunk(keys_s, T, n_chunks, cpb, P, g);
  const int nb = (n_chunks + cpb - 1) / cpb;
  if (P.xrank && (g & ~63) < nb) place_block(keys_s, vals_s, T, cpb, B, P, g, g < nb);
}

template <int G, int J, int CH, int LB1, class Policy>
__device__ __forceinline__ void seg_fold_short(const SegBufs &S, const Policy &pol, int g, int lane, int start, int n, uint32_t prev_key,
                                               uint32_t next_key, bool all_inner, float4 (&acc)[J], float &accs) {
  constexpr int KPL = (2 * CH + G - 1) / G;
  constexpr int LB = J == 1 ? LB1 : (J == 2 ? 4 : 2);
  uint32_t kreg[KPL], vreg[KPL];
#pragma unroll
  for (int q = 0; q < KPL; ++q) {
    const int t = q * G + lane;
    const bool ok = t < n;
    kreg[q] = ok ? S.keys_s[start + t] : DRX_KEY_NONE;
    vreg[q] = ok ? S.vals_s[start + t] : 0u;
  }
  auto bcast = [&](const uint32_t (&reg)[KPL], int t) -> uint32_t {
    uint32_t sel = reg[0];
#pragma unroll
    for (int q = 1; q < KPL; ++q) sel = (t / G == q) ? reg[q] : sel;
    return (uint32_t)__shfl((int)sel, t % G, G);
  };
#pragma unroll
  for (int jx = 0; jx < J; ++jx) acc[jx] = f4_zero();
  accs = 0.f;
  uint32_t cur = DRX_KEY_NONE;
  int cur_pos = 0;
  bool cur_from_start = false;
  auto flush = [&](bool at_end) {
    if (cur == DRX_KEY_NONE) return;
    const bool cont_left = cur_from_start && prev_key == cur;
    const bool cont_right = at_end && next_key == cur;
    if (!cont_left && !cont_right) {
      pol.template finish<G, J>(cur, cur_pos, lane, acc, accs);
    } else if (cont_left) {
      if (!all_inner) {
        store_row<G, J>(S.phead, (size_t)g, S.ld, lane, acc);
        if (lane == 0) S.phs[g] = accs;
      }
    } else {
      store_row<G, J>(S.ptail, (size_t)g, S.ld, lane, acc);
      if (lane == 0) S.pts[g] = accs;
    }
  };
  for (int t0 = 0; t0 < n; t0 += LB) {
    uint32_t k8[LB];
    float s8[LB], c8[LB];
    float4 rows[LB][J];
#pragma unroll
    for (int u = 0; u < LB; ++u) {
      const int t = t0 + u;
      k8[u] = t < n ? bcast(kreg, t) : DRX_KEY_NONE;
      const uint32_t b = bcast(vreg, t < n ? t : 0);
      s8[u] = 0.f;
      c8[u] = 1.f;
#pragma unroll
      for (int jx = 0; jx < J; ++jx) rows[u][jx] = f4_zero();
      if (k8[u] != DRX_KEY_NONE) pol.template load<G, J>(k8[u], b, lane, rows[u], s8[u], c8[u]);
    }
#pragma unroll
    for (int u = 0; u < LB; ++u) {
      const uint32_t key = k8[u];
      if (key != DRX_KEY_NONE) {
        if (key != cur) {
          flush(false);
          cur = key;
          cur_from_start = (t0 + u == 0);
#pragma unroll
          for (int jx = 0; jx < J; ++jx) acc[jx] = f4_zero();
          accs = 0.f;
        }
#pragma unroll
        for (int jx = 0; jx < J; ++jx) f4_fma(acc[jx], c8[u], rows[u][jx]);
        accs += s8[u];
        cur_pos = start + t0 + u;
// ... 97 lines not shown
        k8[0] = lk[t0]; k8[1] = lk[t0 + 1]; b8[0] = lv[t0]; b8[1] = lv[t0 + 1];
      }
      if (cur != DRX_KEY_NONE && k8[0] == cur && k8[LB - 1] == cur) {
        float s8[LB], c8[LB];
        float4 rows[LB][J];
#pragma unroll
        for (int u = 0; u < LB; ++u) {
          s8[u] = 0.f; c8[u] = 1.f;
          pol.template load<G, J>(cur, b8[u], lane, rows[u], s8[u], c8[u]);
        }
#pragma unroll
        for (int u = 0; u < LB; ++u) {
#pragma unroll
          for (int jx = 0; jx < J; ++jx) f4_fma(acc[jx], c8[u], rows[u][jx]);
          accs += s8[u];
        }
        cur_pos = start + t0 + LB - 1;
      } else {
        for (int u = 0; u < LB; ++u) {
          const uint32_t key = lk[t0 + u];
          if (key == DRX_KEY_NONE) continue;
          float sv = 0.f, cv = 1.f;
          float4 row[J];
          pol.template load<G, J>(key, lv[t0 + u], lane, row, sv, cv);
          if (key != cur) {
            flush(false);
            cur = key;
            cur_from_start = (t0 + u == 0);
#pragma unroll
            for (int jx = 0; jx < J; ++jx) acc[jx] = f4_zero();
            accs = 0.f;
          }
#pragma unroll
          for (int jx = 0; jx < J; ++jx) f4_fma(acc[jx], cv, row[jx]);
          accs += sv;
          cur_pos = start + t0 + u;
        }
      }
    }
    flush(n > 0 && bcast(kreg, n - 1) != DRX_KEY_NONE);
  } else {
    seg_fold_short<G, J, CH, LB1>(S, pol, g, lane, start, n, prev_key, next_key, all_inner, acc, accs);
  }
  if (all_inner) {
    float *sc = seg_lds + (size_t)CPB * S.ld;
    store_row<G, J>(seg_lds, (size_t)r, S.ld, lane, acc);
    if (lane == 0) sc[r] = accs;
    __syncthreads();
    if (r == 0) {
      float4 t[J];
#pragma unroll
      for (int jx = 0; jx < J; ++jx) t[jx] = f4_zero();
      float ts = 0.f;
#pragma unroll 8
      for (int rr = 0; rr < CPB; ++rr) {
        float4 v[J];
        load_row<G, J>(seg_lds, (size_t)rr, S.ld, lane, v);
#pragma unroll
        for (int jx = 0; jx < J; ++jx) f4_add(t[jx], v[jx]);
        ts += sc[rr];
      }
      store_row<G, J>(PB.pblock, (size_t)blk, S.ld, lane, t);
      if (lane == 0) PB.pbs[blk] = ts;
    }
  }
}

template <int G, int J>
__device__ __forceinline__ void span_partial(const SegBufs &S, const PlanBufs &PB, const SpanShape &sh, int cpb, int i, int lane,
                                             float4 (&v)[J], float &sv) {
  if (i < sh.n_lead) {
    const int c = sh.first + i;
    load_row<G, J>(S.phead, (size_t)c, S.ld, lane, v); sv = S.phs[c];
  } else if (i < sh.n_lead + sh.n_blk) {
    const int bb = (sh.first + sh.n_lead) / cpb + (i - sh.n_lead);
    load_row<G, J>(PB.pblock, (size_t)bb, S.ld, lane, v); sv = PB.pbs[bb];
  } else {
    const int c = sh.first + sh.n_lead + sh.n_blk * cpb + (i - sh.n_lead - sh.n_blk);
    load_row<G, J>(S.phead, (size_t)c, S.ld, lane, v); sv = S.phs[c];
  }
}

template <int G, int J, class Policy, class Extra>
__global__ __launch_bounds__(kFixBlock) void k_span_planned(SegBufs S, PlanBufs PB, SpanPlan SP, Policy pol, int n_long_blocks,
                                                            int n_short_blocks, Extra extra) {
  extern __shared__ __align__(16) float span_lds[];
  constexpr int R = kFixBlock / G, CPB = kSegBlock / G;
  const int lane = threadIdx.x % G, r = threadIdx.x / G;
  constexpr int UL = J == 1 ? 8 : 2;
  if ((int)blockIdx.x >= n_long_blocks + n_short_blocks) { extra(span_lds); return; }
  if ((int)blockIdx.x >= n_long_blocks) {
    const uint32_t n_short = SP.cnt[0];
    for (uint32_t si = ((int)blockIdx.x - n_long_blocks) * R + r; si < n_short; si += (uint32_t)n_short_blocks * R) {
      const uint2 d = SP.desc[si];
      const SpanShape sh(d, CPB);
      const int g0 = (int)d.x, tot = sh.total();
      const int kpos = min(S.T, (g0 + 1) * SP.chunk) - 1;
      float4 t[J];
      load_row<G, J>(S.ptail, (size_t)g0, S.ld, lane, t);
      float ts = S.pts[g0];
      for (int i0 = 0; i0 < tot; i0 += UL) {
        float4 v[UL][J];
        float sv[UL];
#pragma unroll
        for (int u = 0; u < UL; ++u) {
          sv[u] = 0.f;
#pragma unroll
          for (int j = 0; j < J; ++j) v[u][j] = f4_zero();
          if (i0 + u < tot) span_partial<G, J>(S, PB, sh, CPB, i0 + u, lane, v[u], sv[u]);
        }
#pragma unroll
        for (int u = 0; u < UL; ++u) {
#pragma unroll
          for (int j = 0; j < J; ++j) f4_add(t[j], v[u][j]);
          ts += sv[u];
        }
      }
      pol.template finish<G, J>(S.keys_s[kpos], kpos, lane, t, ts);
    }
    return;
  }
  float *sc = span_lds + (size_t)R * S.ld;
  const uint32_t n_long = SP.cnt[1];
  for (uint32_t si = blockIdx.x; si < n_long; si += (uint32_t)n_long_blocks) {
    const uint2 d = SP.desc[S.n_chunks - 1 - (int)si];
    const SpanShape sh(d, CPB);
    const int g0 = (int)d.x, tot = sh.total();
    const int kpos = min(S.T, (g0 + 1) * SP.chunk) - 1;
    float4 acc[J];
#pragma unroll
    for (int j = 0; j < J; ++j) acc[j] = f4_zero();
    float accs = 0.f;
    const int per = (tot + R - 1) / R;
    const int i_lo = r * per, i_hi = min(tot, i_lo + per);
    for (int i0 = i_lo; i0 < i_hi; i0 += UL) {
      float4 v[UL][J];
      float sv[UL];
#pragma unroll
      for (int u = 0; u < UL; ++u) {
        sv[u] = 0.f;
#pragma unroll
        for (int j = 0; j < J; ++j) v[u][j] = f4_zero();
        if (i0 + u < i_hi) span_partial<G, J>(S, PB, sh, CPB, i0 + u, lane, v[u], sv[u]);
      }
#pragma unroll
      for (int u = 0; u < UL; ++u) {
#pragma unroll
        for (int j = 0; j < J; ++j) f4_add(acc[j], v[u][j]);
        accs += sv[u];
      }
    }
    __syncthreads();
    store_row<G, J>(span_lds, (size_t)r, S.ld, lane, acc);
    if (lane == 0) sc[r] = accs;
    __syncthreads();
    if (r == 0) {
      float4 t[J];
      load_row<G, J>(S.ptail, (size_t)g0, S.ld, lane, t);
      float ts = S.pts[g0];
#pragma unroll 8
      for (int rr = 0; rr < R; ++rr) {
        float4 v[J];
        load_row<G, J>(span_lds, (size_t)rr, S.ld, lane, v);
#pragma unroll
        for (int j = 0; j < J; ++j) f4_add(t[j], v[j]);
        ts += sc[rr];
      }
      pol.template finish<G, J>(S.keys_s[kpos], kpos, lane, t, ts);
    }
  }
}


template <int G, int J, class Policy>
__device__ __forceinline__ void span_short_body(const SegBufs &S, const Policy &pol, int block_id, int n_blocks) {
  const int lane = threadIdx.x % G;
  const int gshift = (threadIdx.x & 63) / G * G;
  const unsigned long long gmask = G == 64 ? ~0ull : ((1ull << G) - 1ull);
  const uint32_t n_span = S.n_span[0];
  const int gpb = kBlock / G;
  constexpr int UL = J == 1 ? 8 : 2;
  for (uint32_t si = block_id * gpb + threadIdx.x / G; si < n_span; si += n_blocks * gpb) {
    const int g0 = (int)S.span_list[si];
    const uint32_t key = S.keys_s[min(S.T, (g0 + 1) * kChunk) - 1];
    int m = 0;
    bool is_long = false;
    for (int base = g0 + 1;; base += G) {
      const int c = base + lane;
      const int fl = c < S.n_chunks ? (int)S.cflag[c] : 0;
      const unsigned long long mid = (__ballot(fl == 2) >> gshift) & gmask;
      const int run = mid == gmask ? G : __builtin_ctzll(~mid);
      m += run;
      if (run < G) {
        m += (__shfl(fl, run, G) == 1) ? 1 : 0;
        break;
      }
      if (m >= kShortSpan) { is_long = true; break; }
    }
    if (is_long || m > kShortSpan) {
      if (lane == 0) S.long_list[atomicAdd(&S.n_span[1], 1u)] = (uint32_t)g0;
      continue;
    }
    float4 t[J];
    load_row<G, J>(S.ptail, (size_t)g0, S.ld, lane, t);
    float ts = S.pts[g0];
    for (int c0 = g0 + 1; c0 <= g0 + m; c0 += UL) {
      float4 v[UL][J];
      float sv[UL];
#pragma unroll
      for (int u = 0; u < UL; ++u) {
        sv[u] = 0.f;
#pragma unroll
        for (int j = 0; j < J; ++j) v[u][j] = f4_zero();
        if (c0 + u <= g0 + m) { load_row<G, J>(S.phead, (size_t)(c0 + u), S.ld, lane, v[u]); sv[u] = S.phs[c0 + u]; }
      }
#pragma unroll
      for (int u = 0; u < UL; ++u) {
#pragma unroll
        for (int j = 0; j < J; ++j) f4_add(t[j], v[u][j]);
        ts += sv[u];
      }
    }
    pol.template finish<G, J>(key, min(S.T, (g0 + 1) * kChunk) - 1, lane, t, ts);
  }
}

template <int G, int J, class Policy>
__global__ __launch_bounds__(kBlock) void k_span_short(SegBufs S, Policy pol) {
  span_short_body<G, J, Policy>(S, pol, (int)blockIdx.x, (int)gridDim.x);
}

template <int G, int J, class Policy>
__device__ __forceinline__ void span_long_body(const SegBufs &S, const Policy &pol, int block_id, int n_blocks, float *lds) {
  constexpr int R = kFixBlock / G;
  float *sc = lds + (size_t)R * S.ld;
  const int lane = threadIdx.x % G, r = threadIdx.x / G;
  const uint32_t n_long = S.n_span[1];
  for (uint32_t si = block_id; si < n_long; si += n_blocks) {
    const int g0 = (int)S.long_list[si];
    const uint32_t key = S.keys_s[min(S.T, (g0 + 1) * kChunk) - 1];
    float4 acc[J];
#pragma unroll
    for (int j = 0; j < J; ++j) acc[j] = f4_zero();
    float accs = 0.f;
    __shared__ int s_stop, s_len;
    int len = 0;
    for (int base = g0 + 1;; base += kFixBlock) {
      if (threadIdx.x == 0) s_stop = kFixBlock;
      __syncthreads();
      const int c = base + (int)threadIdx.x;
      const int fl = c < S.n_chunks ? (int)S.cflag[c] : 0;
      if (fl != 2) atomicMin(&s_stop, (int)threadIdx.x);
      __syncthreads();
// ... 58 lines not shown
```

### drecpy_amd/csrc/drx_segstream.hpp

```cpp
#pragma once
#include "drx_segreduce.hpp"
#include "drx_prep.hpp"

namespace drx {

__device__ __forceinline__ void lds_dma16(const void *gsrc, uint32_t lds_dst) {
  uint32_t keep;
  asm volatile("s_mov_b32 %0, m0\n\ts_mov_b32 m0, %2\n\ts_nop 0\n\tglobal_load_lds_dwordx4 %1, off\n\ts_mov_b32 m0, %0"
               : "=&s"(keep) : "v"(gsrc), "s"(lds_dst) : "memory");
}
template <int N>
__device__ __forceinline__ void wait_vmcnt() { asm volatile("s_waitcnt vmcnt(%0)" :: "n"(N) : "memory"); }

template <int VL> struct LaneVec;
template <> struct LaneVec<1> { using T = float; };
template <> struct LaneVec<2> { typedef float T __attribute__((ext_vector_type(2))); };
template <> struct LaneVec<4> { typedef float T __attribute__((ext_vector_type(4))); };

#ifndef DRX_STREAM_SGPRS
#define DRX_STREAM_SGPRS 80
#endif
#define DRX_STREAM_SGPR_CAP __attribute__((amdgpu_num_sgpr(DRX_STREAM_SGPRS), amdgpu_waves_per_eu(8)))
constexpr int kStreamItems = 3 * (2 * kChunk - 1) + 3;
static inline size_t seg_stream_lds_bytes(int ld, int depth) {
// ... 208 lines not shown
              float *const sf = reinterpret_cast<float *>(&slotv);
#pragma unroll
              for (int v = 0; v < VL; ++v) pol.stream_update(fmaf(decay, pf[v], accf[v]), pf[v], sf[v]);
              const long long roff = (long long)idx * (LD * 4);
              ((GV *)(uintptr_t)(origin + offs[5u * av + kItParam] + roff))[lane] = prow;
              ((GV *)(uintptr_t)(origin + offs[5u * av + kItSlot] + roff))[lane] = slotv;
              float *const spar = av == 0 ? A.sparam[0] : (av == 1 ? A.sparam[1] : A.sparam[2]);
              if (spar) {
                float pb = __builtin_bit_cast(float, __builtin_amdgcn_readlane(__builtin_bit_cast(int, sp), at_lane));
                float ps = __builtin_bit_cast(float, __builtin_amdgcn_readlane(__builtin_bit_cast(int, ss), at_lane));
                pol.stream_update_scalar(accs, pb, ps);
                if (lane == 0) { spar[idx] = pb; (av == 0 ? A.sslot[0] : (av == 1 ? A.sslot[1] : A.sslot[2]))[idx] = ps; }
              }
#pragma unroll
              for (int v = 0; v < VL; ++v) accf[v] = 0.f;
              accs = 0.f;
            }
          }
        }
      }
      if (all_inner) *reinterpret_cast<V *>(comb + (size_t)wv * LD + lane * VL) = acc;
    }
    if (all_inner) {
      float *const sc = comb + (size_t)CPB * LD;
      if (lane == 0) sc[wv] = accs;
      __syncthreads();
      if (wv == 0) {
        V t;
        float *const tf = reinterpret_cast<float *>(&t);
#pragma unroll
        for (int v = 0; v < VL; ++v) tf[v] = 0.f;
        float ts = 0.f;
#pragma unroll
        for (int rr = 0; rr < CPB; ++rr) {
          const V x = *reinterpret_cast<const V *>(comb + (size_t)rr * LD + lane * VL);
          const float *const xf = reinterpret_cast<const float *>(&x);
#pragma unroll
          for (int v = 0; v < VL; ++v) tf[v] += xf[v];
          ts += sc[rr];
        }
        *reinterpret_cast<V *>(PB.pblock + (size_t)blk * LD + lane * VL) = t;
        if (lane == 0) PB.pbs[blk] = ts;
      }
    }
  }
}

template <int G> constexpr int kStreamThreads = (kSegBlock / G) * 64;

template <int G, int J, class Policy, class Front>
static int launch_reduce_streamed(const SegBufs &SB, const PlanBufs &PB, const SpanPlan &plan, const Policy &pol, int n_front,
                                  const Front &front, hipStream_t st) {
  if constexpr (kStreamBuilt<G, J, Policy>) {
    constexpr int cpb = kSegBlock / G;
    hipLaunchKernelGGL((k_seg_reduce_stream<4 * G, kStreamDepth, Policy, Front>), dim3(n_front + (SB.n_chunks + cpb - 1) / cpb),
                       dim3(kStreamThreads<G>), seg_stream_lds_bytes(SB.ld, kStreamDepth), st, SB, PB, plan, pol, n_front, front);
    return DRX_OK;
  }
  return DRX_EINVAL;
}

template <int G, int J, class Policy>
static int launch_reduce(ReduceForm form, const SegBufs &SB, const PlanBufs &PB, const SpanPlan &plan, const Policy &pol,
                         const BiasArgs &BA, hipStream_t st) {
  if (form == ReduceForm::Streamed)
    return launch_reduce_streamed<G, J>(SB, PB, plan, pol, BA.n_part, BiasPartialExtra<G, J, kStreamThreads<G>>{SB.ld, BA}, st);
  constexpr int cpb = kSegBlock / G;
  using Front = BiasPartialExtra<G, J>;
  const bool lng = form == ReduceForm::PlannedLong;
  const auto kernel = lng ? k_seg_reduce_planned<G, J, Policy, true, Front> : k_seg_reduce_planned<G, J, Policy, false, Front>;
  hipLaunchKernelGGL(kernel, dim3(BA.n_part + (SB.n_chunks + cpb - 1) / cpb), dim3(kSegBlock), seg_reduce_lds_bytes(cpb, SB.ld, lng), st,
                     SB, PB, plan, pol, BA.n_part, Front{SB.ld, BA});
  return DRX_OK;
}

constexpr int kSpanBlocks = kLongBlocks + kShortBlocks;
template <int G, int J, class Policy, class Extra>
static int launch_spans(const SegBufs &SB, const PlanBufs &PB, const SpanPlan &plan, const Policy &pol, int n_extra, const Extra &extra,
                        hipStream_t st) {
  const size_t lds = ((size_t)(kFixBlock / G) * (SB.ld + 1)) * 4;
  if (lds > 48 * 1024)
    DRX_HIP(hipFuncSetAttribute((const void *)k_span_planned<G, J, Policy, Extra>, hipFuncAttributeMaxDynamicSharedMemorySize, (int)lds));
  hipLaunchKernelGGL((k_span_planned<G, J, Policy, Extra>), dim3(kSpanBlocks + n_extra), dim3(kFixBlock), lds, st, SB, PB, plan, pol,
                     kLongBlocks, kShortBlocks, extra);
  return DRX_OK;
}

}
```

### drecpy_amd/csrc/drx_shard.hip

```cpp
#include "drx_common.hpp"
#include "drx_rows.hpp"
#include "drx_segreduce.hpp"
#include "drx_scan.hpp"
#include "drx_prep.hpp"
#include "drx_segstream.hpp"

namespace drx {

constexpr int kTileKeys = 8192;
constexpr int kTileWords = kTileKeys / 32;

struct ShardGeo {
  int world, rank, ipr, shift, ld, bypass;
  int chunks, cshift, units;
  uint32_t n_words, n_tiles, tiles_per_unit;
  __host__ __device__ WireGeo wg() const { return WireGeo{ipr, cshift, world}; }
  __host__ __device__ bool own_unit(int v) const { return bypass && v % world == rank; }
};

static int chunks_of(const DrxShard &sh, int shift) {
  int c = sh.chunks < 1 ? 1 : sh.chunks;
  while (c > 1 && (shift - __builtin_ctz((unsigned)c)) < 13) c >>= 1;
  return c;
}
// ... 255 lines not shown
#pragma unroll
        for (int jx = 0; jx < J; ++jx) r[q][jx] = f4_zero();
        if (oq != DRX_KEY_NONE) {
          const float *const cb = S.cache, *const wb = P.W;
          load_row<G, J>(((oq & 0x80000000u) ? wb : cb) + (size_t)(oq & 0x7FFFFFFFu), 0, P.ld, lane, r[q]);
        }
      }
#pragma unroll
      for (int q = 0; q < NF; ++q)
#pragma unroll
        for (int jx = 0; jx < J; ++jx) f4_add(acc[jx], r[q][jx]);
    }
  }
  float4 h[J], w2[J];
  hidden_act<G, J>(P, u, scale, lane, acc, h);
  const int i = bt.iid[b];
  const int oo = i / S.ipr;
  const uint32_t wo = S.G.wire(i, 1);
  const uint32_t po = S.X.pos_of(wo);
  const size_t ro = S.X.row_off(wo, po), sco = S.X.scal_off(wo, po);
  const bool own_out = oo == S.self;
  {
    const float *const cb = S.cache, *const tb = P.W2T;
    load_row<G, J>(own_out ? tb + (size_t)(i - oo * S.ipr) * P.ld : cb + ro, 0, P.ld, lane, w2);
  }
  float d = 0.f;
#pragma unroll
  for (int j = 0; j < J; ++j) d += f4_dot(w2[j], h[j]);
  d = group_sum<G>(d);
  const float y = bt.y[b];
  const float p = sigmoidf_(d + (own_out ? P.b2[i - oo * S.ipr] : S.cache[sco]));
  const float invB = 1.0f / (float)S.b_norm;
  float lval, dp;
  if (loss_kind == DRX_LOSS_BCE) { lval = bce_elem(y, p); dp = bce_grad(y, p) * invB; }
  else { lval = (p - y) * (p - y); dp = 2.0f * (p - y) * invB; }
  const float dz2 = dp * p * (1.0f - p);
  float4 dz1[J], g2[J];
#pragma unroll
  for (int j = 0; j < J; ++j) {
    dz1[j].x = dz2 * w2[j].x * h[j].x * (1.0f - h[j].x); dz1[j].y = dz2 * w2[j].y * h[j].y * (1.0f - h[j].y);
    dz1[j].z = dz2 * w2[j].z * h[j].z * (1.0f - h[j].z); dz1[j].w = dz2 * w2[j].w * h[j].w * (1.0f - h[j].w);
    g2[j].x = dz2 * h[j].x; g2[j].y = dz2 * h[j].y; g2[j].z = dz2 * h[j].z; g2[j].w = dz2 * h[j].w;
  }
  store_row<G, J>(S.dz1, (size_t)b, P.ld, lane, dz1);
  if (lane == 0) S.lossb[b] = lval;
  const bool solo_v = S.solo_v && S.solo_v[b], solo_o = S.solo_o && S.solo_o[b];
  if (solo_o) {
    store_row<G, J>(S.gsend + ro, 0, P.ld, lane, g2);
    if (lane == 0) S.gsend[sco] = dz2;
  } else {
    store_row<G, J>(S.g2, (size_t)b, P.ld, lane, g2);
    if (lane == 0) S.dz2[b] = dz2;
  }
  if (solo_v) {
    OptScalars o = opt_for(opt, 0, S.b_norm);
    o.inv_k = 1.0f / (float)P.k;
    float4 w[J];
    load_row<G, J>(P.V, (size_t)u, P.ld, lane, w);
    row_update<G, J, KIND>(o, P.V, opt.s1[2], opt.s2[2], (size_t)u, P.ld, lane, w, dz1);
  }
}

template <int KIND>
struct LocalPolicyT {
  DrxCdaeParams P;
  DrxOptim opt;
  int b_norm, n_items, ipr;
  float scale;
  const float *dz1;
  long long g2_off;
  const float *dz2;
  float *gsend;
  ShardXfer X;
  WireGeo WG;
  template <int G, int J>
  __device__ __forceinline__ void load(uint32_t key, uint32_t b, int lane, float4 (&row)[J], float &sc, float &coef) const {
    const uint32_t N = (uint32_t)n_items;
    const bool is_out = key >= N && key < 2 * N;
    load_row<G, J>(dz1 + (is_out ? g2_off : 0ll), (size_t)b, P.ld, lane, row);
    if (is_out) sc = dz2[b];
    coef = key < N ? scale : 1.0f;
  }
  template <int G, int J>
  __device__ __forceinline__ void finish(uint32_t key, int, int lane, const float4 (&g)[J], float gs) const {
    const uint32_t N = (uint32_t)n_items;
    if (key >= 2 * N) {
      const size_t row = key - 2 * N;
      OptScalars o = opt_for(opt, 0, b_norm);
      o.inv_k = 1.0f / (float)P.k;
      float4 w[J];
      load_row<G, J>(P.V, row, P.ld, lane, w);
      row_update<G, J, KIND>(o, P.V, opt.s1[2], opt.s2[2], row, P.ld, lane, w, g);
    } else {
      const bool is_out = key >= N;
      const int item = (int)(is_out ? key - N : key);
      const uint32_t w = WG.wire(item, is_out ? 1 : 0);
      const uint32_t pos = X.pos_of(w);
      store_row<G, J>(gsend + X.row_off(w, pos), 0, P.ld, lane, g);
      if (is_out && lane == 0) gsend[X.scal_off(w, pos)] = gs;
    }
  }
  static constexpr bool kStreamParks = true;
  __device__ __forceinline__ StreamArrays stream_arrays() const {
    const uint32_t N = (uint32_t)n_items;
    return StreamArrays{{0u, N, 2u * N}, {dz1, dz1 + g2_off, dz1}, {nullptr, nullptr, P.V}, {nullptr, nullptr, opt.s1[2]},
                        {scale, 1.0f, 1.0f}, {nullptr, dz2, nullptr}, {nullptr, nullptr, nullptr}, {nullptr, nullptr, nullptr}};
  }
  __device__ __forceinline__ bool stream_parked(uint32_t av) const { return av < 2u; }
  __device__ __forceinline__ void stream_park_at(uint32_t av, uint32_t item, uint32_t &roff, uint32_t &soff) const {
    const uint32_t w = WG.wire((int)item, av == 1u ? 1 : 0);
    const uint32_t pos = X.pos_of(w);
    roff = (uint32_t)X.row_off(w, pos);
    soff = (uint32_t)X.scal_off(w, pos);
  }
  __device__ __forceinline__ float *stream_park_base() const { return gsend; }
  __device__ __forceinline__ float stream_decay() const { return opt.reg_rate / (float)b_norm; }
  __device__ __forceinline__ void stream_update(float g, float &p, float &a) const {
    static_assert(KIND == DRX_OPT_ADAGRAD || KIND < 0, "one slot per element");
    OptScalars o = opt_for(opt, 0, b_norm);
    float unused = 0.f;
    opt_update1<DRX_OPT_ADAGRAD>(o, g, p, a, unused);
  }
  __device__ __forceinline__ void stream_update_scalar(float g, float &p, float &a) const { stream_update(g, p, a); }
};

template <int G, int J>
struct ShardBiasExtra {
  int ld, units;
  BiasArgs A;
  float *gsend;
  ShardXfer X;
  __device__ __forceinline__ void operator()(float *lds) const {
    __shared__ float red[kFixBlock / 64];
    constexpr int R = kFixBlock / G;
    const int lane = threadIdx.x % G, r = threadIdx.x / G;
    float4 acc[J];
#pragma unroll
    for (int j = 0; j < J; ++j) acc[j] = f4_zero();
    constexpr int NB = J == 1 ? 8 : 2;
    for (int i = r; i < A.n_part; i += NB * R) {
      float4 v[NB][J];
#pragma unroll
      for (int q = 0; q < NB; ++q) {
#pragma unroll
        for (int j = 0; j < J; ++j) v[q][j] = f4_zero();
        if (i + q * R < A.n_part) load_row<G, J>(A.part, (size_t)(i + q * R), ld, lane, v[q]);
      }
#pragma unroll
      for (int q = 0; q < NB; ++q)
#pragma unroll
        for (int j = 0; j < J; ++j) f4_add(acc[j], v[q][j]);
    }
    store_row<G, J>(lds, (size_t)r, ld, lane, acc);
    __syncthreads();
    const float *lp = A.part + (size_t)A.n_part * ld;
    float a = 0.f;
    for (int i = threadIdx.x; i < A.n_part; i += kFixBlock) a += lp[i];
    const float tl = block_sum(a, red);
    if (r == 0) {
      float4 g[J];
#pragma unroll
      for (int j = 0; j < J; ++j) g[j] = f4_zero();
#pragma unroll 8
      for (int rr = 0; rr < R; ++rr) {
        float4 v[J];
        load_row<G, J>(lds, (size_t)rr, ld, lane, v);
#pragma unroll
        for (int j = 0; j < J; ++j) f4_add(g[j], v[j]);
      }
      for (int v = 0; v < units; ++v) {
        store_row<G, J>(gsend + X.sentinel_row(v), 0, ld, lane, g);
        if (threadIdx.x == 0) gsend[X.sentinel_scal(v)] = tl;
      }
    }
  }
};

template <int G, int J, int KIND>
static __global__ __launch_bounds__(kBlock) void k_shard_apply(DrxCdaeParams P, DrxOptim opt, ShardGeo g, int b_norm, SegOff so,
                                                               const uint32_t *__restrict__ recv_keys, int n,
                                                               const uint32_t *__restrict__ tab, const float *__restrict__ grecv,
                                                               int row_blocks, float *loss_out, int do_bias) {
  const int lane = threadIdx.x % G;
  const int gpb = kBlock / G;
  const int W = so.n_seg;
  if ((int)blockIdx.x >= row_blocks) {
    if (do_bias && threadIdx.x < G) {
      float4 gb[J], w[J];
#pragma unroll
      for (int j = 0; j < J; ++j) gb[j] = f4_zero();
      float ls = 0.f;
      for (int s = 0; s < W; ++s) {
        const int m = so.koff[s + 1] - so.koff[s], i = m - 1;
        const float *ch = so.chunk(grecv, s);
        float4 v[J];
        load_row<G, J>(ch + (size_t)i * P.ld, 0, P.ld, lane, v);
#pragma unroll
        for (int j = 0; j < J; ++j) f4_add(gb[j], v[j]);
        ls += ch[(size_t)m * P.ld + i];
      }
      load_row<G, J>(P.b, 0, P.ld, lane, w);
      OptScalars o = opt_for(opt, 0, b_norm);
      if (o.kind == DRX_OPT_ROWWISE_ADAGRAD) o.kind = DRX_OPT_ADAGRAD;
      o.rb = 0.f;
      row_update<G, J>(o, P.b, opt.s1[3], opt.s2[3], 0, P.ld, lane, w, gb);
      if (threadIdx.x == 0 && loss_out) { loss_out[0] = ls / (float)b_norm; loss_out[1] = 0.f; }
    }
    return;
  }
  constexpr int NR = J == 1 ? 4 : 2;
  for (int j0 = (blockIdx.x * gpb + threadIdx.x / G) * NR; j0 < n; j0 += row_blocks * gpb * NR) {
    uint32_t lk[NR];
    bool live[NR];
    float4 gsum[NR][J];
    float gs[NR];
    if (W == 1) {
      const float *ch = so.chunk(grecv, 0);
      const int m = so.koff[1];
#pragma unroll
      for (int q = 0; q < NR; ++q) {
        const int j = j0 + q;
        const uint32_t key = j < n ? recv_keys[j] : DRX_KEY_NONE;
        live[q] = key != DRX_KEY_NONE;
        lk[q] = g.wg().local(key);
        gs[q] = 0.f;
#pragma unroll
        for (int jx = 0; jx < J; ++jx) gsum[q][jx] = f4_zero();
        if (live[q]) {
          load_row<G, J>(ch + (size_t)j * P.ld, 0, P.ld, lane, gsum[q]);
          gs[q] = ch[(size_t)m * P.ld + j];
        }
      }
    } else {
#pragma unroll
      for (int q = 0; q < NR; ++q) {
        const int j = j0 + q;
        const uint32_t key = j < n ? recv_keys[j] : DRX_KEY_NONE;
        live[q] = key != DRX_KEY_NONE;
        lk[q] = g.wg().local(key);
        gs[q] = 0.f;
#pragma unroll
// ... 375 lines not shown
```

### include/drx.h

```cpp
#ifndef DRX_H_
#define DRX_H_

#include <stddef.h>
#include <stdint.h>

#ifdef __cplusplus
extern "C" {
#endif

#define DRX_VERSION 100

enum {
  DRX_OK = 0,
  DRX_EINVAL = -1,
  DRX_ESCRATCH = -2,
  DRX_ENOTIMPL = -3,
  DRX_ERETRY = -4,
  DRX_ECOMM = -5
};

#define DRX_MAX_K 1024
#define DRX_KEY_NONE 0xFFFFFFFFu

enum { DRX_LOSS_BCE = 0, DRX_LOSS_MSE = 1 };
// ... 44 lines not shown
  uint32_t flags;
} DrxBatch;
#define DRX_BATCH_SHARE_USERS 1u

typedef struct DrxOptim {
  int32_t kind;
  float lr, reg_rate;
  float beta1, beta2, eps;
  float alpha[5];
  float *s1[5];
  float *s2[5];
} DrxOptim;

int drx_version(void);
const char *drx_strerror(int code);

void *drx_event_create(void);
void drx_event_destroy(void *ev);
int drx_event_record(void *ev, void *stream);
int drx_stream_wait_event(void *stream, void *ev);
int drx_event_synchronize(void *ev);

void *drx_stream_create_cu_slice(int32_t cus_per_xcd);
void drx_stream_destroy(void *stream);

uint32_t drx_hash_u32(uint64_t seed, uint32_t a, uint32_t b);

int drx_cdae_forward(const DrxCdaeParams *p, const DrxHistory *hist, const DrxBatch *bt,
                     float *h, float *pred, void *stream);

size_t drx_cdae_scratch_bytes(const DrxCdaeParams *p, int32_t B, int32_t n_touch_slots, int32_t dense_mode);

int drx_cdae_step_dense(const DrxCdaeParams *p, const DrxOptim *opt, const DrxHistory *hist,
                        const DrxBatch *bt, int32_t loss_kind, int32_t targets_kind,
                        void *scratch, size_t scratch_bytes, float *loss_out, void *stream);

int drx_cdae_step_sparse(const DrxCdaeParams *p, const DrxOptim *opt, const DrxHistory *hist,
                         const DrxBatch *bt, int32_t loss_kind,
                         void *scratch, size_t scratch_bytes, float *loss_out, void *stream);

#define DRX_SPARSE_PHASES 5
int drx_cdae_step_sparse_timed(const DrxCdaeParams *p, const DrxOptim *opt, const DrxHistory *hist,
                               const DrxBatch *bt, int32_t loss_kind, void *scratch, size_t scratch_bytes,
                               float *loss_out, void *const *events, void *stream);

size_t drx_cdae_prep_bytes(const DrxCdaeParams *p, int32_t B, int32_t n_touch_slots);
int drx_cdae_sparse_prepare(const DrxCdaeParams *p, const DrxHistory *hist, const DrxBatch *bt, void *prepared,
                            size_t prepared_bytes, void *stream);
int drx_cdae_step_sparse_prepared(const DrxCdaeParams *p, const DrxOptim *opt, const DrxHistory *hist, const DrxBatch *bt,
                                  int32_t loss_kind, const void *prepared, size_t prepared_bytes, void *scratch,
                                  size_t scratch_bytes, float *loss_out, void *const *events, void *stream);

typedef struct DrxHotHead {
  int32_t H;
  const int16_t *slot;
  const int32_t *item;
} DrxHotHead;
#define DRX_MAX_HOT 1024
size_t drx_cdae_prep_bytes_hot(const DrxCdaeParams *p, int32_t B, int32_t n_touch_slots, int32_t H);
size_t drx_cdae_scratch_bytes_hot(const DrxCdaeParams *p, int32_t B, int32_t n_touch_slots, int32_t H);
int drx_cdae_sparse_prepare_hot(const DrxCdaeParams *p, const DrxHistory *hist, const DrxBatch *bt, const DrxHotHead *hot,
                                void *prepared, size_t prepared_bytes, void *stream);
int drx_cdae_step_sparse_hot(const DrxCdaeParams *p, const DrxOptim *opt, const DrxHistory *hist, const DrxBatch *bt,
                             const DrxHotHead *hot, int32_t loss_kind, const void *prepared, size_t prepared_bytes, void *scratch,
                             size_t scratch_bytes, float *loss_out, void *const *events, void *stream);
int32_t drx_cdae_hot_rows_for(const DrxCdaeParams *p, int32_t opt_kind, int32_t B, int32_t n_touch_slots, int32_t H);
void drx_cdae_prep_forget(const void *prepared);

int drx_debug_prep_counts(const DrxCdaeParams *p, const DrxHistory *hist, const DrxBatch *bt, const DrxHotHead *hot, uint8_t *present,
                          int32_t ipr, int32_t cshift, int32_t world, void *prepared, size_t prepared_bytes, uint32_t *hist_out,
                          uint32_t *buckets_out, uint32_t *keys_out, uint32_t *vals_out, uint32_t *mask_out, int32_t *info_out,
                          void *stream);

int drx_debug_prep_result(const DrxCdaeParams *p, int32_t B, int32_t n_touch_slots, int32_t H, const void *prepared, size_t prepared_bytes,
                          uint32_t *keys_s_out, uint32_t *vals_s_out, uint8_t *solo_v_out, uint8_t *solo_o_out, int32_t *order_out,
                          void *stream);

int drx_debug_cdae_reduce(const DrxCdaeParams *p, const DrxOptim *opt, const DrxHistory *hist, const DrxBatch *bt, const DrxHotHead *hot,
                          const void *prepared, size_t prepared_bytes, const float *dz1_in, const float *g2_in, const float *dz2_in,
                          int32_t form, void *scratch, size_t scratch_bytes, void *stream);

int drx_debug_span_plan(const DrxCdaeParams *p, int32_t B, int32_t n_touch_slots, int32_t H, const void *prepared, size_t prepared_bytes,
                        uint8_t *ext_out, uint32_t *desc_out, uint32_t *cnt_out, void *stream);

int drx_batch_offsets(const int64_t *indptr, const int32_t *ids, int32_t B, int32_t *off, void *scratch, size_t scratch_bytes, void *stream);

size_t drx_point_sample_scratch_bytes(int32_t B);
int drx_point_sample(const DrxHistory *hist, int32_t n_users, int32_t n_items, int32_t B, int32_t neg_ratio,
                     uint64_t seed, int32_t *uid, int32_t *iid, float *y, int32_t *keep_off,
                     void *scratch, size_t scratch_bytes, uint64_t *host_mailbox, uint32_t tag, void *stream);
int drx_point_sample_recorded(const DrxHistory *hist, const DrxHistory *recorded, int32_t n_users, int32_t n_items, int32_t B,
                              int32_t neg_ratio, uint64_t seed, int32_t *uid, int32_t *iid, float *y, int32_t *keep_off,
                              void *scratch, size_t scratch_bytes, uint64_t *host_mailbox, uint32_t tag, void *stream);

size_t drx_point_sample_by_user_scratch_bytes(int32_t B, int32_t n_users);
int drx_point_sample_by_user(const DrxHistory *hist, const DrxHistory *recorded, int32_t n_users, int32_t n_items, int32_t B,
                             int32_t neg_ratio, uint64_t seed, int32_t *uid, int32_t *iid, float *y, int32_t *keep_off, void *scratch,
                             size_t scratch_bytes, uint64_t *host_mailbox, uint32_t tag, void *stream);

int drx_point_sample_valued(const DrxHistory *hist, const DrxHistory *recorded, const float *pos_values, float vmin, float vrange,
                            int32_t n_users, int32_t n_items, int32_t B, int32_t neg_ratio, uint64_t seed, int32_t *uid, int32_t *iid,
                            float *y, void *stream);

typedef struct DrxListGroups {
  const int64_t *indptr;
  const int32_t *seq_ids;
  const int64_t *held_indptr;
  const int32_t *held;
  const int32_t *group_value;
  const int32_t *eligible;
  int32_t n_groups, n_eligible, n_ids;
} DrxListGroups;
int drx_list_sample_device(const DrxListGroups *g, int32_t B, int32_t n_inputs, int32_t n_targets, int32_t neg_ratio, uint64_t seed,
                           int32_t *group_out, int32_t *before, int32_t *after, void *stream);

int drx_cdae_kshard_forward(const DrxCdaeParams *p, const DrxHistory *hist, const DrxBatch *bt, float *h_out ,
                            float *dot_partial , void *stream);
int drx_cdae_kshard_forward_prepared(const DrxCdaeParams *p, const DrxHistory *hist, const DrxBatch *bt, const void *prepared,
                                     size_t prepared_bytes, float *h_out , float *dot_partial , void *stream);
int drx_cdae_kshard_step(const DrxCdaeParams *p, const DrxOptim *opt, const DrxHistory *hist, const DrxBatch *bt, int32_t loss_kind,
                         const float *h, const float *dot_total, const void *prepared, size_t prepared_bytes, void *scratch,
                         size_t scratch_bytes, float *loss_out, void *const *events, void *stream);

size_t drx_cdae_prep_result_bytes(const DrxCdaeParams *p, int32_t B, int32_t n_touch_slots);

size_t drx_cdae_prep_part_out_bytes(const DrxCdaeParams *p, int32_t B, int32_t n_touch_slots, int32_t parts);
int drx_cdae_prep_part_layout(const DrxCdaeParams *p, int32_t B, int32_t n_touch_slots, int32_t parts, size_t *out4);
size_t drx_cdae_prep_part_bytes(const DrxCdaeParams *p, int32_t B, int32_t n_touch_slots, int32_t parts);
int drx_cdae_sparse_prepare_part(const DrxCdaeParams *p, const DrxHistory *hist, const DrxBatch *bt, int32_t part, int32_t parts,
                                 void *part_out, size_t part_out_bytes, void *scratch, size_t scratch_bytes, void *stream);
int drx_cdae_sparse_prepare_assemble(const DrxCdaeParams *p, const DrxBatch *bt, const void *all_parts, int32_t parts, void *prepared,
                                     size_t prepared_bytes, int32_t *overflow_out, void *stream);

#define DRX_MAX_WORLD 64
#define DRX_MAX_MICRO 4
#define DRX_MAX_CHUNKS 16
typedef struct DrxShard {
  int32_t world, rank;
  int32_t n_items;
  int32_t items_per_rank;
  int32_t n_users_local;
  uint32_t flags;
  int32_t chunks;
} DrxShard;
int32_t drx_shard_chunks(const DrxShard *sh);
int32_t drx_shard_unit_shift(const DrxShard *sh);
#define DRX_SHARD_SELF_BYPASS 1u

size_t drx_shard_prep_bytes(const DrxCdaeParams *p, const DrxShard *sh, int32_t B, int32_t n_touch_slots);
size_t drx_shard_work_bytes(const DrxShard *sh);
int drx_shard_prep_layout(const DrxCdaeParams *p, const DrxShard *sh, int32_t B, int32_t n_touch_slots, size_t *out4);
int drx_shard_prepare(const DrxCdaeParams *p, const DrxShard *sh, const DrxHistory *hist, const DrxBatch *bt, void *prepared,
                      size_t prepared_bytes, void *work, size_t work_bytes, void *stream);
size_t drx_shard_owner_table_bytes(const DrxShard *sh, int32_t n_segments);
int drx_shard_owner_index(const DrxShard *sh, const uint32_t *recv_keys, int32_t n, const int32_t *recv_counts, int32_t n_segments,
                          int32_t chunk, void *table, size_t table_bytes, void *stream);
int drx_shard_gather_rows(const DrxCdaeParams *p, const DrxShard *sh, const uint32_t *recv_keys, int32_t n, const int32_t *recv_counts,
                          int32_t n_segments, float *out, void *stream);
size_t drx_shard_step_scratch_bytes(const DrxCdaeParams *p, int32_t B, int32_t n_touch_slots);
int drx_shard_step_local(const DrxCdaeParams *p, const DrxOptim *opt, const DrxShard *sh, const DrxHistory *hist, const DrxBatch *bt,
                         const void *prepared, size_t prepared_bytes, const float *rows_cache, float *grad_send, int32_t b_norm,
                         int32_t loss_kind, void *scratch, size_t scratch_bytes, void *const *events, void *stream);
int drx_shard_apply(const DrxCdaeParams *p, const DrxOptim *opt, const DrxShard *sh, int32_t b_norm, const uint32_t *recv_keys,
                    const float *grad_recv, int32_t n, const int32_t *recv_counts, int32_t n_segments, int32_t chunk, const void *table,
                    const float *const *own_grad, const int64_t *own_off, float *loss_out, void *stream);

// ... 385 lines not shown
```

Measured before the change: 218.0 million samples/s.

## Prefetch span keys and optimizer rows ahead of segment reduction in span kernel

Adds a per-chunk key array to the span plan so each span workgroup reads its destination key directly and prefetches the next descriptor and key during the current iteration. The extra workgroups (bias finish and hot-row finish) are moved to the front of the grid, and they issue their parameter and optimizer-slot loads before the reduction barrier. Loss partial loads are also issued early. A row-first fetch/finish_loaded path is added, but it is compiled off (kRowFirst=false). The goal is to hide global-memory latency in the sparse update tail, at the cost of more register pressure and a plan-building dependency on the new key array.

Result: no change. 217.7 million samples/s (-0.1%).

```diff
diff --git a/drecpy_amd/_lib.py b/drecpy_amd/_lib.py
--- a/drecpy_amd/_lib.py
+++ b/drecpy_amd/_lib.py
@@ -175,6 +175,8 @@
                                         C.c_void_p]),
     'drx_debug_span_plan': (C.c_int, [C.POINTER(CdaeParams), C.c_int32, C.c_int32, C.c_int32, C.c_void_p, C.c_size_t, C.c_void_p,
                                       C.c_void_p, C.c_void_p, C.c_void_p]),
+    'drx_debug_span_keys': (C.c_int, [C.POINTER(CdaeParams), C.c_int32, C.c_int32, C.c_int32, C.c_void_p, C.c_size_t, C.c_void_p,
+                                      C.c_void_p]),
     'drx_cdae_step_sparse_hot': (C.c_int, [C.POINTER(CdaeParams), C.POINTER(Optim), C.POINTER(History), C.POINTER(Batch),
                                            C.POINTER(HotHead), C.c_int32, C.c_void_p, C.c_size_t, C.c_void_p, C.c_size_t,
                                            C.c_void_p, C.POINTER(C.c_void_p), C.c_void_p]),
diff --git a/drecpy_amd/csrc/drx_cdae.hip b/drecpy_amd/csrc/drx_cdae.hip
--- a/drecpy_amd/csrc/drx_cdae.hip
+++ b/drecpy_amd/csrc/drx_cdae.hip
@@ -34,30 +34,69 @@
   int T, n_chunks, n_bpart;
 };
 
-template <int G, int J, int KIND = -1>
-__device__ __forceinline__ void sparse_apply(const DrxCdaeParams &P, const DrxOptim &opt, int B, uint32_t key, int lane,
-                                             const float4 (&g)[J], float gs) {
+struct SparseRowAt {
+  float *tab, *s1, *s2;
+  size_t row;
+  int var;
+};
+__device__ __forceinline__ SparseRowAt sparse_row_at(const DrxCdaeParams &P, const DrxOptim &opt, uint32_t key) {
   const uint32_t N = (uint32_t)P.n_items;
   float *const tW = P.W, *const tO = P.W2T, *const tV = P.V;
   float *const a0 = opt.s1[0], *const a1 = opt.s1[1], *const a2 = opt.s1[2];
   float *const c0 = opt.s2[0], *const c1 = opt.s2[1], *const c2 = opt.s2[2];
   const int var = key < N ? 0 : (key < 2 * N ? 1 : 2);
-  const size_t row = key - (uint32_t)var * N;
-  float *const tab = var == 0 ? tW : (var == 1 ? tO : tV);
-  float *const s1 = var == 0 ? a0 : (var == 1 ? a1 : a2);
-  float *const s2 = var == 0 ? c0 : (var == 1 ? c1 : c2);
+  return SparseRowAt{var == 0 ? tW : (var == 1 ? tO : tV), var == 0 ? a0 : (var == 1 ? a1 : a2), var == 0 ? c0 : (var == 1 ? c1 : c2),
+                     (size_t)(key - (uint32_t)var * N), var};
+}
+
+template <int G, int J, int KIND = -1>
+__device__ __forceinline__ void sparse_fetch(const DrxCdaeParams &P, const DrxOptim &opt, uint32_t key, int lane, SegRow<J> &R) {
+  const SparseRowAt at = sparse_row_at(P, opt, key);
+  R.tab = at.tab; R.s1 = at.s1; R.s2 = at.s2; R.at = at.row; R.var = at.var;
+  OptScalars o = opt_for(opt, 0, 1);
+  load_row<G, J>(at.tab, at.row, P.ld, lane, R.w);
+  row_slots<G, J, KIND>(o, at.s1, at.s2, at.row, P.ld, lane, R.m, R.v);
+  R.pb = R.mb = R.vb = 0.f;
+  if (at.var == 1 && lane == 0) {
+    const int kind = KIND >= 0 ? KIND : o.kind;
+    R.pb = P.b2[at.row];
+    R.mb = opt.s1[4][at.row];
+    if (kind == DRX_OPT_ADAM) R.vb = opt.s2[4][at.row];
+  }
+}
+
+template <int G, int J, int KIND = -1>
+__device__ __forceinline__ void sparse_update(const DrxCdaeParams &P, const DrxOptim &opt, int B, int lane, const float4 (&g)[J], float gs,
+                                              const SegRow<J> &R) {
+  OptScalars o = opt_for(opt, 0, B);
+  o.inv_k = 1.0f / (float)P.k;
+  row_update_loaded<G, J, KIND>(o, R.tab, R.s1, R.s2, R.at, P.ld, lane, R.w, R.m, R.v, g);
+  if (R.var == 1 && lane == 0) {
+    const int kind = KIND >= 0 ? KIND : o.kind;
+    float pb = R.pb, m = R.mb, v = R.vb;
+    o.rb = 0.f;
+    opt_update1<KIND>(o, gs, pb, m, v);
+    P.b2[R.at] = pb; opt.s1[4][R.at] = m;
+    if (kind == DRX_OPT_ADAM) opt.s2[4][R.at] = v;
+  }
+}
+
+template <int G, int J, int KIND = -1>
+__device__ __forceinline__ void sparse_apply(const DrxCdaeParams &P, const DrxOptim &opt, int B, uint32_t key, int lane,
+                                             const float4 (&g)[J], float gs) {
+  const SparseRowAt at = sparse_row_at(P, opt, key);
   OptScalars o = opt_for(opt, 0, B);
   o.inv_k = 1.0f / (float)P.k;
   float4 w[J];
-  load_row<G, J>(tab, row, P.ld, lane, w);
-  row_update<G, J, KIND>(o, tab, s1, s2, row, P.ld, lane, w, g);
-  if (var == 1 && lane == 0) {
+  load_row<G, J>(at.tab, at.row, P.ld, lane, w);
+  row_update<G, J, KIND>(o, at.tab, at.s1, at.s2, at.row, P.ld, lane, w, g);
+  if (at.var == 1 && lane == 0) {
     const int kind = KIND >= 0 ? KIND : o.kind;
-    float pb = P.b2[row], m = opt.s1[4][row], v = kind == DRX_OPT_ADAM ? opt.s2[4][row] : 0.f;
+    float pb = P.b2[at.row], m = opt.s1[4][at.row], v = kind == DRX_OPT_ADAM ? opt.s2[4][at.row] : 0.f;
     o.rb = 0.f;
     opt_update1<KIND>(o, gs, pb, m, v);
-    P.b2[row] = pb; opt.s1[4][row] = m;
-    if (kind == DRX_OPT_ADAM) opt.s2[4][row] = v;
+    P.b2[at.row] = pb; opt.s1[4][at.row] = m;
+    if (kind == DRX_OPT_ADAM) opt.s2[4][at.row] = v;
   }
 }
 
@@ -380,6 +419,14 @@
   __device__ __forceinline__ void finish(uint32_t key, int, int lane, const float4 (&g)[J], float gs) const {
     sparse_apply<G, J, KIND>(P, opt, B, key, lane, g, gs);
   }
+  template <int G, int J>
+  __device__ __forceinline__ void fetch(uint32_t key, int lane, SegRow<J> &R) const {
+    sparse_fetch<G, J, KIND>(P, opt, key, lane, R);
+  }
+  template <int G, int J>
+  __device__ __forceinline__ void finish_loaded(uint32_t key, int, int lane, const float4 (&g)[J], float gs, const SegRow<J> &R) const {
+    sparse_update<G, J, KIND>(P, opt, B, lane, g, gs, R);
+  }
   static constexpr bool kStreamParks = false;
   __device__ __forceinline__ StreamArrays stream_arrays() const {
     const uint32_t N = (uint32_t)P.n_items;
@@ -400,12 +447,18 @@
 
 template <int G, int J, int NT>
 __device__ __forceinline__ void bias_final_body(const DrxCdaeParams &P, const DrxOptim &opt, const BiasArgs &A,
-                                                float *lds , float *red) {
+                                                float *lds , float *red, unsigned long long *stamps) {
   constexpr int R = NT / G;
   const int lane = threadIdx.x % G, r = threadIdx.x / G;
   float4 acc[J];
 #pragma unroll
   for (int j = 0; j < J; ++j) acc[j] = f4_zero();
+  OptScalars which{};
+  which.kind = opt.kind == DRX_OPT_ROWWISE_ADAGRAD ? DRX_OPT_ADAGRAD : opt.kind;
+  float4 w[J], m[J], v2[J];
+  const float *lp = A.part + (size_t)A.n_part * P.ld;
+  StridedPair lq{0.f, 0.f};
+  if (A.loss_out) lq = strided_ask<NT>(lp, A.n_part);
   constexpr int NB = J == 1 ? 8 : 2;
   for (int i = r; i < A.n_part; i += NB * R) {
     float4 v[NB][J];
@@ -420,10 +473,17 @@
 #pragma unroll
       for (int j = 0; j < J; ++j) f4_add(acc[j], v[q][j]);
   }
+  if (r == 0) {
+    load_row<G, J>(P.b, 0, P.ld, lane, w);
+    row_slots<G, J>(which, opt.s1[3], opt.s2[3], 0, P.ld, lane, m, v2);
+  }
   store_row<G, J>(lds, (size_t)r, P.ld, lane, acc);
+#ifdef DRX_STAMPS
+  if (acc[0].x == acc[0].x) DRX_SPAN_STAMP(stamps, 1);
+#endif
   __syncthreads();
   if (r == 0) {
-    float4 g[J], w[J];
+    float4 g[J];
 #pragma unroll
     for (int j = 0; j < J; ++j) g[j] = f4_zero();
 #pragma unroll 8
@@ -433,17 +493,13 @@
 #pragma unroll
       for (int j = 0; j < J; ++j) f4_add(g[j], v[j]);
     }
-    load_row<G, J>(P.b, 0, P.ld, lane, w);
     OptScalars o = opt_for(opt, 0, A.B);
-    if (o.kind == DRX_OPT_ROWWISE_ADAGRAD) o.kind = DRX_OPT_ADAGRAD;
+    o.kind = which.kind;
     o.rb = 0.f;
-    row_update<G, J>(o, P.b, opt.s1[3], opt.s2[3], 0, P.ld, lane, w, g);
+    row_update_loaded<G, J>(o, P.b, opt.s1[3], opt.s2[3], 0, P.ld, lane, w, m, v2, g);
   }
   if (A.loss_out) {
-    const float *lp = A.part + (size_t)A.n_part * P.ld;
-    float a = 0.f;
-    for (int b = threadIdx.x; b < A.n_part; b += NT) a += lp[b];
-    float t = block_sum(a, red);
+    float t = block_sum(strided_sum<NT>(lp, A.n_part, lq), red);
     if (threadIdx.x == 0) { A.loss_out[0] = t / (float)A.B; A.loss_out[1] = 0.f; }
   }
 }
@@ -453,9 +509,9 @@
   DrxCdaeParams P;
   DrxOptim opt;
   BiasArgs A;
-  __device__ __forceinline__ void operator()(float *lds) const {
+  __device__ __forceinline__ void operator()(float *lds, unsigned long long *stamps) const {
     __shared__ float red[kFixBlock / 64];
-    bias_final_body<G, J, kFixBlock>(P, opt, A, lds, red);
+    bias_final_body<G, J, kFixBlock>(P, opt, A, lds, red, stamps);
   }
 };
 
@@ -580,33 +636,45 @@
   }
 };
 
+constexpr int kHotFlight = 32;
 template <int LD, class Policy>
 struct HotFinishExtra {
   HotArgs A;
   Policy pol;
-  __device__ __forceinline__ void operator()(float *lds) const {
+  __device__ __forceinline__ void operator()(float *lds, unsigned long long *stamps) const {
     constexpr int NT = kFixBlock, NQ = NT / LD;
     static_assert(NQ >= 1 && NT % LD == 0, "a row per workgroup");
     const int h = (int)blockIdx.x - A.first;
     if (h >= A.H) return;
+    const int c = (int)threadIdx.x % LD, q = (int)threadIdx.x / LD;
+    const StreamArrays SA = pol.stream_arrays();
+    const size_t off = (size_t)A.item[h] * LD + c;
     const uint32_t bit = 1u << (h & 31);
-    bool touched = false;
-    for (int s = (int)threadIdx.x; s < A.S; s += NT) touched |= (A.any[(size_t)s * (A.H / 32) + (h >> 5)] & bit) != 0u;
-    if (!__syncthreads_or(touched)) return;
-    const int c = (int)threadIdx.x % LD, q = (int)threadIdx.x / LD;
+    uint32_t flags = 0u;
+    for (int s = (int)threadIdx.x; s < A.S; s += NT) flags |= A.any[(size_t)s * (A.H / 32) + (h >> 5)];
     const int per = (A.S + NQ - 1) / NQ, s0 = q * per, s1 = min(A.S, s0 + per);
-    float sum = 0.f;
-#pragma unroll 8
-    for (int s = s0; s < s1; ++s) sum += A.part[((size_t)s * A.H + h) * LD + c];
+    const float *const col = A.part + (size_t)h * LD + c;
+    const size_t sstride = (size_t)A.H * LD;
+    float sum = 0.f, pv = 0.f, av = 0.f;
+    for (int sb = s0; sb < s1; sb += kHotFlight) {
+      float x[kHotFlight];
+#pragma unroll
+      for (int u = 0; u < kHotFlight; ++u) x[u] = sb + u < s1 ? col[(size_t)(sb + u) * sstride] : 0.f;
+      if (sb == s0 && q == 0) { pv = SA.table[0][off]; av = SA.slot[0][off]; }
+#pragma unroll
+      for (int u = 0; u < kHotFlight; ++u)
+        if (sb + u < s1) sum += x[u];
+    }
     lds[q * LD + c] = sum;
-    __syncthreads();
+#ifdef DRX_STAMPS
+    if (sum == sum) DRX_SPAN_STAMP(stamps, 1);
+    if (pv == pv && av == av) DRX_SPAN_STAMP(stamps, 2);
+#endif
+    if (!__syncthreads_or((flags & bit) != 0u)) return;
     if (q == 0) {
       float t = lds[c];
 #pragma unroll
       for (int k = 1; k < NQ; ++k) t += lds[k * LD + c];
-      const StreamArrays SA = pol.stream_arrays();
-      const size_t off = (size_t)A.item[h] * LD + c;
-      float pv = SA.table[0][off], av = SA.slot[0][off];
       pol.stream_update(fmaf(pol.stream_decay(), pv, A.scale * t), pv, av);
       SA.table[0][off] = pv;
       SA.slot[0][off] = av;
@@ -619,9 +687,9 @@
   E1 e1;
   int n1;
   E2 e2;
-  __device__ __forceinline__ void operator()(float *lds) const {
-    if ((int)blockIdx.x < n1) e1(lds);
-    else e2(lds);
+  __device__ __forceinline__ void operator()(float *lds, unsigned long long *stamps) const {
+    if ((int)blockIdx.x < n1) e1(lds, stamps);
+    else e2(lds, stamps);
   }
 };
 
@@ -722,7 +790,7 @@
   if (HA.H == 0) rc = launch_spans<G, J>(SB, PB, plan, pol, 1, bias, st);
   else if constexpr (kHotBuilt<G, J, Policy>) {
     HotArgs fin = HA;
-    fin.first = kSpanBlocks + 1;
+    fin.first = 1;
     using Finish = ExtraPair<BiasFinalExtra<G, J>, HotFinishExtra<4 * G, Policy>>;
     rc = launch_spans<G, J>(SB, PB, plan, pol, 1 + HA.H, Finish{bias, fin.first, {fin, pol}}, st);
   }
@@ -1058,6 +1126,18 @@
   return DRX_OK;
 }
 
+int drx_debug_span_keys(const DrxCdaeParams *p, int32_t B, int32_t n_touch_slots, int32_t H, const void *prepared, size_t prepared_bytes,
+                        uint32_t *key_out, void *stream) {
+  int rc = check_params(p);
+  if (rc) return rc;
+  if (B < 1 || n_touch_slots < 0 || hot_rows(p, H) < 0 || !prepared || !key_out) return DRX_EINVAL;
+  Carver cp(const_cast<void *>(prepared), prepared_bytes);
+  const PrepBufs R = prep_layout(cp, *p, B, n_touch_slots, H);
+  if (!cp.ok()) return DRX_ESCRATCH;
+  DRX_HIP(hipMemcpyAsync(key_out, R.plan.key, (size_t)R.n_chunks * sizeof(uint32_t), hipMemcpyDeviceToDevice, (hipStream_t)stream));
+  return DRX_OK;
+}
+
 int drx_cdae_step_sparse_hot(const DrxCdaeParams *p, const DrxOptim *opt, const DrxHistory *hist, const DrxBatch *bt,
                              const DrxHotHead *hot, int32_t loss_kind, const void *prepared, size_t prepared_bytes, void *scratch,
                              size_t scratch_bytes, float *loss_out, void *const *events, void *stream) {
diff --git a/drecpy_amd/csrc/drx_common.hpp b/drecpy_amd/csrc/drx_common.hpp
--- a/drecpy_amd/csrc/drx_common.hpp
+++ b/drecpy_amd/csrc/drx_common.hpp
@@ -107,6 +107,7 @@
 #else
 #define DRX_STAMP(buf, unit, i, lane) do { } while (0)
 #endif
+#define DRX_SPAN_STAMP(buf, i) DRX_STAMP(buf, blockIdx.x, 8 + (i), threadIdx.x)
 
 inline size_t align_up(size_t x, size_t a) { return (x + a - 1) / a * a; }
 
diff --git a/drecpy_amd/csrc/drx_prep.hpp b/drecpy_amd/csrc/drx_prep.hpp
--- a/drecpy_amd/csrc/drx_prep.hpp
+++ b/drecpy_amd/csrc/drx_prep.hpp
@@ -494,6 +494,7 @@
   R.plan.chunk = seg_chunk(long_segments(R.T, P));
   R.n_chunks = (R.T + R.plan.chunk - 1) / R.plan.chunk;
   R.plan.desc = cv.take<uint2>(R.n_chunks);
+  R.plan.key = cv.take<uint32_t>(R.n_chunks);
   R.plan.cnt = cv.take<uint32_t>(128);
   R.plan.ext = cv.take<uint8_t>(R.n_chunks);
   {
diff --git a/drecpy_amd/csrc/drx_rows.hpp b/drecpy_amd/csrc/drx_rows.hpp
--- a/drecpy_amd/csrc/drx_rows.hpp
+++ b/drecpy_amd/csrc/drx_rows.hpp
@@ -186,6 +186,92 @@
   }
 }
 
+template <int J>
+struct SegRow {
+  float4 w[J], m[J], v[J];
+  float pb, mb, vb;
+  float *tab, *s1, *s2;
+  size_t at;
+  int var;
+};
+
+template <int G, int J, int KIND = -1>
+__device__ __forceinline__ void row_slots(const OptScalars &o, const float *s1, const float *s2, size_t row, int ld, int lane,
+                                          float4 (&m)[J], float4 (&v)[J]) {
+  const int kind = KIND >= 0 ? KIND : o.kind;
+#pragma unroll
+  for (int j = 0; j < J; ++j) m[j] = v[j] = f4_zero();
+  if (kind == DRX_OPT_ROWWISE_ADAGRAD) {
+    m[0].x = s1[row * (size_t)ld];
+    return;
+  }
+  const float4 *a1 = reinterpret_cast<const float4 *>(s1 + row * (size_t)ld);
+  const float4 *a2 = (kind == DRX_OPT_ADAM) ? reinterpret_cast<const float4 *>(s2 + row * (size_t)ld) : nullptr;
+#pragma unroll
+  for (int j = 0; j < J; ++j) {
+    const int c = lane + j * G;
+    if (4 * c < ld) {
+      m[j] = a1[c];
+      if (a2) v[j] = a2[c];
+    }
+  }
+}
+
+template <int G, int J, int KIND = -1>
+__device__ __forceinline__ float row_update_loaded(const OptScalars &o, float *tab, float *s1, float *s2, size_t row, int ld, int lane,
+                                                   const float4 (&w)[J], const float4 (&m0)[J], const float4 (&v0)[J],
+                                                   const float4 (&g)[J]) {
+  float sq = 0.f;
+  float4 *pr = reinterpret_cast<float4 *>(tab + row * (size_t)ld);
+  const int kind = KIND >= 0 ? KIND : o.kind;
+  if (kind == DRX_OPT_ROWWISE_ADAGRAD) {
+    float4 gg[J];
+    float q = 0.f;
+#pragma unroll
+    for (int j = 0; j < J; ++j) {
+      const float4 p = w[j];
+      gg[j].x = fmaf(o.rb, p.x, g[j].x); gg[j].y = fmaf(o.rb, p.y, g[j].y);
+      gg[j].z = fmaf(o.rb, p.z, g[j].z); gg[j].w = fmaf(o.rb, p.w, g[j].w);
+      q += f4_dot(gg[j], gg[j]);
+      sq += f4_dot(p, p);
+    }
+    q = group_sum<G>(q) * o.inv_k;
+    const float acc = m0[0].x + q;
+    const float step = o.lr / (sqrtf(acc) + o.eps);
+#pragma unroll
+    for (int j = 0; j < J; ++j) {
+      const int c = lane + j * G;
+      if (4 * c < ld) {
+        float4 p = w[j];
+        p.x -= step * gg[j].x; p.y -= step * gg[j].y; p.z -= step * gg[j].z; p.w -= step * gg[j].w;
+        pr[c] = p;
+      }
+    }
+    if (lane == 0) s1[row * (size_t)ld] = acc;
+    return sq;
+  }
+  float4 *a1 = reinterpret_cast<float4 *>(s1 + row * (size_t)ld);
+  float4 *a2 = (kind == DRX_OPT_ADAM) ? reinterpret_cast<float4 *>(s2 + row * (size_t)ld) : nullptr;
+#pragma unroll
+  for (int j = 0; j < J; ++j) {
+    const int c = lane + j * G;
+    if (4 * c < ld) {
+      float4 p = w[j];
+      float4 m = m0[j];
+      float4 v = v0[j];
+      sq += f4_dot(p, p);
+      opt_update1<KIND>(o, fmaf(o.rb, p.x, g[j].x), p.x, m.x, v.x);
+      opt_update1<KIND>(o, fmaf(o.rb, p.y, g[j].y), p.y, m.y, v.y);
+      opt_update1<KIND>(o, fmaf(o.rb, p.z, g[j].z), p.z, m.z, v.z);
+      opt_update1<KIND>(o, fmaf(o.rb, p.w, g[j].w), p.w, m.w, v.w);
+      pr[c] = p;
+      a1[c] = m;
+      if (a2) a2[c] = v;
+    }
+  }
+  return sq;
+}
+
 template <int G, int J, int KIND = -1>
 __device__ __forceinline__ float row_update(const OptScalars &o, float *tab, float *s1, float *s2, size_t row, int ld,
                                             int lane, const float4 (&w)[J], const float4 (&g)[J]) {
@@ -258,4 +344,20 @@
   return t;
 }
 
-}
+struct StridedPair { float x0, x1; };
+template <int NT>
+__device__ __forceinline__ StridedPair strided_ask(const float *x, int n) {
+  const int t = (int)threadIdx.x;
+  return StridedPair{t < n ? x[t] : 0.f, t + NT < n ? x[t + NT] : 0.f};
+}
+template <int NT>
+__device__ __forceinline__ float strided_sum(const float *x, int n, const StridedPair &p) {
+  const int t = (int)threadIdx.x;
+  float a = 0.f;
+  if (t < n) a += p.x0;
+  if (t + NT < n) a += p.x1;
+  for (int i = t + 2 * NT; i < n; i += NT) a += x[i];
+  return a;
+}
+
+}
diff --git a/drecpy_amd/csrc/drx_segreduce.hpp b/drecpy_amd/csrc/drx_segreduce.hpp
--- a/drecpy_amd/csrc/drx_segreduce.hpp
+++ b/drecpy_amd/csrc/drx_segreduce.hpp
@@ -143,6 +143,7 @@
   int chunk;
   const int32_t *row_end;
   uint32_t row_end_keys;
+  uint32_t *key;
 };
 #ifndef DRX_STREAM_PLACED
 #define DRX_STREAM_PLACED 0
@@ -273,8 +274,10 @@
     return;
   }
   const uint2 d = make_uint2((uint32_t)g, m_in | (has_end << 31));
-  if (SpanShape(d, cpb).total() <= kPlanShort) P.desc[atomicAdd(&P.cnt[0], 1u)] = d;
-  else P.desc[n_chunks - 1 - (int)atomicAdd(&P.cnt[1], 1u)] = d;
+  const bool is_short = SpanShape(d, cpb).total() <= kPlanShort;
+  const int at = is_short ? (int)atomicAdd(&P.cnt[0], 1u) : n_chunks - 1 - (int)atomicAdd(&P.cnt[1], 1u);
+  P.desc[at] = d;
+  P.key[at] = last;
 }
 
 template <int DUMMY = 0>
@@ -538,57 +541,92 @@
 }
 
 template <int G, int J, class Policy, class Extra>
-__global__ __launch_bounds__(kFixBlock) void k_span_planned(SegBufs S, PlanBufs PB, SpanPlan SP, Policy pol, int n_long_blocks,
-                                                            int n_short_blocks, Extra extra) {
+__global__ __launch_bounds__(kFixBlock) void k_span_planned(SegBufs S, PlanBufs PB, SpanPlan SP, Policy pol, int n_extra,
+                                                            int n_long_blocks, int n_short_blocks, Extra extra) {
   extern __shared__ __align__(16) float span_lds[];
   constexpr int R = kFixBlock / G, CPB = kSegBlock / G;
   const int lane = threadIdx.x % G, r = threadIdx.x / G;
   constexpr int UL = J == 1 ? 8 : 2;
-  if ((int)blockIdx.x >= n_long_blocks + n_short_blocks) { extra(span_lds); return; }
-  if ((int)blockIdx.x >= n_long_blocks) {
+  constexpr int US = UL;
+  constexpr bool kRowFirst = false;
+  const int wg = (int)blockIdx.x - n_extra;
+  DRX_SPAN_STAMP(S.stamps, 0);
+  if (wg < 0) {
+    extra(span_lds, S.stamps);
+    DRX_SPAN_STAMP(S.stamps, 6);
+    return;
+  }
+  if (wg >= n_long_blocks) {
+    uint32_t si = (uint32_t)(wg - n_long_blocks) * R + r;
+    const bool in = si < (uint32_t)S.n_chunks;
+    uint2 d = in ? SP.desc[si] : make_uint2(0u, 0u);
+    uint32_t key = in ? SP.key[si] : DRX_KEY_NONE;
     const uint32_t n_short = SP.cnt[0];
-    for (uint32_t si = ((int)blockIdx.x - n_long_blocks) * R + r; si < n_short; si += (uint32_t)n_short_blocks * R) {
-      const uint2 d = SP.desc[si];
+    while (si < n_short) {
       const SpanShape sh(d, CPB);
       const int g0 = (int)d.x, tot = sh.total();
       const int kpos = min(S.T, (g0 + 1) * SP.chunk) - 1;
+#ifdef DRX_STAMPS
+      if (g0 >= 0) DRX_SPAN_STAMP(S.stamps, 1);
+#endif
+      SegRow<J> row;
+      if constexpr (kRowFirst) pol.template fetch<G, J>(key, lane, row);
       float4 t[J];
       load_row<G, J>(S.ptail, (size_t)g0, S.ld, lane, t);
       float ts = S.pts[g0];
-      for (int i0 = 0; i0 < tot; i0 += UL) {
-        float4 v[UL][J];
-        float sv[UL];
-#pragma unroll
-        for (int u = 0; u < UL; ++u) {
+      for (int i0 = 0; i0 < tot; i0 += US) {
+        float4 v[US][J];
+        float sv[US];
+#pragma unroll
+        for (int u = 0; u < US; ++u) {
           sv[u] = 0.f;
 #pragma unroll
           for (int j = 0; j < J; ++j) v[u][j] = f4_zero();
           if (i0 + u < tot) span_partial<G, J>(S, PB, sh, CPB, i0 + u, lane, v[u], sv[u]);
         }
 #pragma unroll
-        for (int u = 0; u < UL; ++u) {
+        for (int u = 0; u < US; ++u) {
 #pragma unroll
           for (int j = 0; j < J; ++j) f4_add(t[j], v[u][j]);
           ts += sv[u];
         }
       }
-      pol.template finish<G, J>(S.keys_s[kpos], kpos, lane, t, ts);
-    }
+#ifdef DRX_STAMPS
+      if (t[0].x == t[0].x && (!kRowFirst || row.w[0].x == row.w[0].x)) DRX_SPAN_STAMP(S.stamps, 2);
+#endif
+      if constexpr (kRowFirst) pol.template finish_loaded<G, J>(key, kpos, lane, t, ts, row);
+      else pol.template finish<G, J>(key, kpos, lane, t, ts);
+      si += (uint32_t)n_short_blocks * R;
+      if (si < n_short) { d = SP.desc[si]; key = SP.key[si]; }
+    }
+    DRX_SPAN_STAMP(S.stamps, 6);
     return;
   }
   float *sc = span_lds + (size_t)R * S.ld;
+  uint32_t si = (uint32_t)wg;
+  const bool in = si < (uint32_t)S.n_chunks;
+  uint2 d = in ? SP.desc[S.n_chunks - 1 - (int)si] : make_uint2(0u, 0u);
+  uint32_t key = in ? SP.key[S.n_chunks - 1 - (int)si] : DRX_KEY_NONE;
   const uint32_t n_long = SP.cnt[1];
-  for (uint32_t si = blockIdx.x; si < n_long; si += (uint32_t)n_long_blocks) {
-    const uint2 d = SP.desc[S.n_chunks - 1 - (int)si];
+  while (si < n_long) {
     const SpanShape sh(d, CPB);
     const int g0 = (int)d.x, tot = sh.total();
     const int kpos = min(S.T, (g0 + 1) * SP.chunk) - 1;
-    float4 acc[J];
-#pragma unroll
-    for (int j = 0; j < J; ++j) acc[j] = f4_zero();
-    float accs = 0.f;
+#ifdef DRX_STAMPS
+    if (g0 >= 0) DRX_SPAN_STAMP(S.stamps, 1);
+#endif
+    float4 acc[J], t[J];
+#pragma unroll
+    for (int j = 0; j < J; ++j) acc[j] = t[j] = f4_zero();
+    float accs = 0.f, ts = 0.f;
+    SegRow<J> row;
     const int per = (tot + R - 1) / R;
     const int i_lo = r * per, i_hi = min(tot, i_lo + per);
+    if (r == 0) {
+      if constexpr (kRowFirst) pol.template fetch<G, J>(key, lane, row);
+      load_row<G, J>(S.ptail, (size_t)g0, S.ld, lane, t);
+      ts = S.pts[g0];
+    }
     for (int i0 = i_lo; i0 < i_hi; i0 += UL) {
       float4 v[UL][J];
       float sv[UL];
@@ -606,14 +644,15 @@
         accs += sv[u];
       }
     }
+#ifdef DRX_STAMPS
+    if (acc[0].x == acc[0].x && t[0].x == t[0].x && (!kRowFirst || row.w[0].x == row.w[0].x)) DRX_SPAN_STAMP(S.stamps, 2);
+#endif
     __syncthreads();
     store_row<G, J>(span_lds, (size_t)r, S.ld, lane, acc);
     if (lane == 0) sc[r] = accs;
     __syncthreads();
+    DRX_SPAN_STAMP(S.stamps, 3);
     if (r == 0) {
-      float4 t[J];
-      load_row<G, J>(S.ptail, (size_t)g0, S.ld, lane, t);
-      float ts = S.pts[g0];
 #pragma unroll 8
       for (int rr = 0; rr < R; ++rr) {
         float4 v[J];
@@ -622,9 +661,13 @@
         for (int j = 0; j < J; ++j) f4_add(t[j], v[j]);
         ts += sc[rr];
       }
-      pol.template finish<G, J>(S.keys_s[kpos], kpos, lane, t, ts);
-    }
-  }
+      if constexpr (kRowFirst) pol.template finish_loaded<G, J>(key, kpos, lane, t, ts, row);
+      else pol.template finish<G, J>(key, kpos, lane, t, ts);
+    }
+    si += (uint32_t)n_long_blocks;
+    if (si < n_long) { d = SP.desc[S.n_chunks - 1 - (int)si]; key = SP.key[S.n_chunks - 1 - (int)si]; }
+  }
+  DRX_SPAN_STAMP(S.stamps, 6);
 }
 
 
diff --git a/drecpy_amd/csrc/drx_segstream.hpp b/drecpy_amd/csrc/drx_segstream.hpp
--- a/drecpy_amd/csrc/drx_segstream.hpp
+++ b/drecpy_amd/csrc/drx_segstream.hpp
@@ -314,7 +314,7 @@
   if (lds > 48 * 1024)
     DRX_HIP(hipFuncSetAttribute((const void *)k_span_planned<G, J, Policy, Extra>, hipFuncAttributeMaxDynamicSharedMemorySize, (int)lds));
   hipLaunchKernelGGL((k_span_planned<G, J, Policy, Extra>), dim3(kSpanBlocks + n_extra), dim3(kFixBlock), lds, st, SB, PB, plan, pol,
-                     kLongBlocks, kShortBlocks, extra);
+                     n_extra, kLongBlocks, kShortBlocks, extra);
   return DRX_OK;
 }
 
diff --git a/drecpy_amd/csrc/drx_shard.hip b/drecpy_amd/csrc/drx_shard.hip
--- a/drecpy_amd/csrc/drx_shard.hip
+++ b/drecpy_amd/csrc/drx_shard.hip
@@ -361,6 +361,25 @@
     coef = key < N ? scale : 1.0f;
   }
   template <int G, int J>
+  __device__ __forceinline__ void fetch(uint32_t key, int lane, SegRow<J> &R) const {
+    const uint32_t N = (uint32_t)n_items;
+    if (key < 2 * N) return;
+    const size_t row = key - 2 * N;
+    load_row<G, J>(P.V, row, P.ld, lane, R.w);
+    row_slots<G, J, KIND>(opt_for(opt, 0, b_norm), opt.s1[2], opt.s2[2], row, P.ld, lane, R.m, R.v);
+  }
+  template <int G, int J>
+  __device__ __forceinline__ void finish_loaded(uint32_t key, int pos, int lane, const float4 (&g)[J], float gs, const SegRow<J> &R) const {
+    const uint32_t N = (uint32_t)n_items;
+    if (key >= 2 * N) {
+      OptScalars o = opt_for(opt, 0, b_norm);
+      o.inv_k = 1.0f / (float)P.k;
+      row_update_loaded<G, J, KIND>(o, P.V, opt.s1[2], opt.s2[2], key - 2 * N, P.ld, lane, R.w, R.m, R.v, g);
+    } else {
+      finish<G, J>(key, pos, lane, g, gs);
+    }
+  }
+  template <int G, int J>
   __device__ __forceinline__ void finish(uint32_t key, int, int lane, const float4 (&g)[J], float gs) const {
     const uint32_t N = (uint32_t)n_items;
     if (key >= 2 * N) {
@@ -409,13 +428,15 @@
   BiasArgs A;
   float *gsend;
   ShardXfer X;
-  __device__ __forceinline__ void operator()(float *lds) const {
+  __device__ __forceinline__ void operator()(float *lds, unsigned long long *) const {
     __shared__ float red[kFixBlock / 64];
     constexpr int R = kFixBlock / G;
     const int lane = threadIdx.x % G, r = threadIdx.x / G;
     float4 acc[J];
 #pragma unroll
     for (int j = 0; j < J; ++j) acc[j] = f4_zero();
+    const float *lp = A.part + (size_t)A.n_part * ld;
+    const StridedPair lq = strided_ask<kFixBlock>(lp, A.n_part);
     constexpr int NB = J == 1 ? 8 : 2;
     for (int i = r; i < A.n_part; i += NB * R) {
       float4 v[NB][J];
@@ -432,10 +453,7 @@
     }
     store_row<G, J>(lds, (size_t)r, ld, lane, acc);
     __syncthreads();
-    const float *lp = A.part + (size_t)A.n_part * ld;
-    float a = 0.f;
-    for (int i = threadIdx.x; i < A.n_part; i += kFixBlock) a += lp[i];
-    const float tl = block_sum(a, red);
+    const float tl = block_sum(strided_sum<kFixBlock>(lp, A.n_part, lq), red);
     if (r == 0) {
       float4 g[J];
 #pragma unroll
diff --git a/include/drx.h b/include/drx.h
--- a/include/drx.h
+++ b/include/drx.h
@@ -150,6 +150,9 @@
 
 int drx_debug_span_plan(const DrxCdaeParams *p, int32_t B, int32_t n_touch_slots, int32_t H, const void *prepared, size_t prepared_bytes,
                         uint8_t *ext_out, uint32_t *desc_out, uint32_t *cnt_out, void *stream);
+
+int drx_debug_span_keys(const DrxCdaeParams *p, int32_t B, int32_t n_touch_slots, int32_t H, const void *prepared, size_t prepared_bytes,
+                        uint32_t *key_out, void *stream);
 
 int drx_batch_offsets(const int64_t *indptr, const int32_t *ids, int32_t B, int32_t *off, void *scratch, size_t scratch_bytes, void *stream);
 
```
